# Aikku93/ulc-codec

Measured on AMD Instinct MI355X. Metric: encode+decode Msamples/s at BlockSize=2048 stereo (channel-samples through encode+decode, VBR -50, 32 blocks per stream per call), higher is better.
Workload: dtype f32; 1 GPU; vbr50 (configs[1] encode, configs[2] decode): Batch=4096 independent 44.1 kHz stereo streams/GPU x 32 blocks, BlockSize=2048, VBR -50; step = encode then decode; config=vbr50, mode=both, streams_per_gpu=4096, block_size=2048, channels=2, parallelism=batch split over 1 GPU(s), no collective on the data path

## Files before the change

### include/ulc_amd.h

```cpp
#ifndef ULC_AMD_H
#define ULC_AMD_H
#include <stddef.h>
#include <stdint.h>

#ifdef __cplusplus
extern "C" {
#endif

#ifndef ULC_AMD_NO_DROPIN_TYPES
struct ULC_TransientData_t { float Sum, SumW; };

struct ULC_EncoderState_t {
    int    RateHz;
    int    nChan;
    int    BlockSize;
    int    WindowCtrl;
    int    NextWindowCtrl;
    float  BlockComplexity;
    float  TransientFilter[3];
    void  *BufferData;
    float *SampleBuffer;
    float *TransformBuffer;
    float *TransformNoise;
    float *TransformFwdLap;
// ... 118 lines not shown
int  ulcx_encoder_reset_streams_dev(ulcx_encoder *enc, const int32_t *d_slots, int n, void *hipStream);
int  ulcx_encoder_save_streams_dev (ulcx_encoder *enc, const int32_t *d_slots, int n, uint8_t *d_state, void *hipStream);
int  ulcx_encoder_load_streams_dev (ulcx_encoder *enc, const int32_t *d_slots, int n, const uint8_t *d_state, void *hipStream);
int  ulcx_decoder_reset_streams_dev(ulcx_decoder *dec, const int32_t *d_slots, int n, void *hipStream);
int  ulcx_decoder_save_streams_dev (ulcx_decoder *dec, const int32_t *d_slots, int n, uint8_t *d_state, void *hipStream);
int  ulcx_decoder_load_streams_dev (ulcx_decoder *dec, const int32_t *d_slots, int n, const uint8_t *d_state, void *hipStream);
int  ulcx_encode_dev_subset      (ulcx_encoder *enc, const int32_t *d_slots, int n, int mode, float param0, float param1,
                                  const ulcx_rate *d_rate, const float *d_pcm , int nBlocks,
                                  uint8_t *d_out , int32_t *d_bits, int32_t *d_wc, float *d_cplx, void *hipStream);
int  ulcx_encode_dev_pcm16_subset(ulcx_encoder *enc, const int32_t *d_slots, int n, int mode, float param0, float param1,
                                  const ulcx_rate *d_rate, const int16_t *d_pcm16, int nBlocks,
                                  uint8_t *d_out, int32_t *d_bits, int32_t *d_wc, float *d_cplx, void *hipStream);
int  ulcx_analyse_dev_subset     (ulcx_encoder *enc, const int32_t *d_slots, int n, const float *d_pcm, int nBlocks,
                                  int32_t *d_wc, float *d_cplx, void *hipStream);
int  ulcx_decode_dev_subset      (ulcx_decoder *dec, const int32_t *d_slots, int n, const uint8_t *d_in ,
                                  int slotBytes, int nBlocks, float *d_pcm, int32_t *d_bits, void *hipStream);
int  ulcx_decode_dev_pcm16_subset(ulcx_decoder *dec, const int32_t *d_slots, int n, const uint8_t *d_in,
                                  int slotBytes, int nBlocks, int16_t *d_pcm16, int32_t *d_bits, void *hipStream);
int  ulcx_encoder_reset_streams_host(ulcx_encoder *enc, const int32_t *h_slots, int n);
int  ulcx_encoder_save_streams_host (ulcx_encoder *enc, const int32_t *h_slots, int n, uint8_t *h_state);
int  ulcx_encoder_load_streams_host (ulcx_encoder *enc, const int32_t *h_slots, int n, const uint8_t *h_state);
int  ulcx_decoder_reset_streams_host(ulcx_decoder *dec, const int32_t *h_slots, int n);
int  ulcx_decoder_save_streams_host (ulcx_decoder *dec, const int32_t *h_slots, int n, uint8_t *h_state);
int  ulcx_decoder_load_streams_host (ulcx_decoder *dec, const int32_t *h_slots, int n, const uint8_t *h_state);
int  ulcx_encode_host_subset(ulcx_encoder *enc, const int32_t *h_slots, int n, int mode, float param0, float param1,
                             const ulcx_rate *h_rate, const float *h_pcm, int nBlocks,
                             uint8_t *h_out, int32_t *h_bits, int32_t *h_wc, float *h_cplx);
int  ulcx_decode_host_subset(ulcx_decoder *dec, const int32_t *h_slots, int n, const uint8_t *h_in, int slotBytes, int nBlocks,
                             float *h_pcm, int32_t *h_bits);
#define ULCX_STATE_MAGIC_ENC 0x45535855u
#define ULCX_STATE_MAGIC_DEC 0x44535855u

#define ULCX_ULC_MAGIC 0x32434C55u
typedef struct ulcx_file_header {
    uint32_t Magic;
    uint16_t BlockSize;
    uint16_t MaxBlockSize;
    uint32_t nBlocks;
    uint32_t RateHz;
    uint16_t nChan;
    uint16_t RateKbps;
    uint32_t StreamOffs;
} ulcx_file_header;
void ulcx_ulc_header_pack(uint8_t dst[24], const ulcx_file_header *h);
int  ulcx_ulc_header_parse(ulcx_file_header *h, const uint8_t *src, size_t len);
int  ulcx_ulc_rate_kbps(uint64_t totalBytes, uint32_t RateHz, uint32_t BlockSize, uint32_t nBlocks);

int  ulcx_pack_streams_dev(int device, int nStreams, int nBlocks, int slotBytes, const uint8_t *d_slots, const int32_t *d_bits,
                           uint8_t *d_payload, long long payloadStride, int32_t *d_payloadBytes, int32_t *d_maxBlock, void *hipStream);

int  ulcx_decode_packed_dev(ulcx_decoder *dec, const uint8_t *d_payload, long long payloadStride, const int32_t *d_payloadBytes,
                            int nBlocks, float *d_pcm, int32_t *d_bits, void *hipStream);
int  ulcx_decode_packed_host(ulcx_decoder *dec, const uint8_t *h_payload, long long payloadStride, const int32_t *h_payloadBytes,
                             int nBlocks, float *h_pcm, int32_t *h_bits);

int  ulcx_decoder_upload_payload(ulcx_decoder *dec, const uint8_t *h_payload, long long payloadStride, const int32_t *h_payloadBytes);
int  ulcx_decode_resident_host(ulcx_decoder *dec, int nBlocks, float *h_pcm, int32_t *h_bits);

typedef struct ulcx_index_entry { int32_t ByteOffs; uint32_t RngState; } ulcx_index_entry;
int  ulcx_index_packed_dev(ulcx_decoder *dec, const uint8_t *d_payload, long long payloadStride, const int32_t *d_payloadBytes,
                           int maxBlocks, ulcx_index_entry *d_index , int32_t *d_nBlocks ,
                           void *hipStream);
int  ulcx_index_packed_host(ulcx_decoder *dec, const uint8_t *h_payload, long long payloadStride, const int32_t *h_payloadBytes,
                            int maxBlocks, ulcx_index_entry *h_index, int32_t *h_nBlocks);
int  ulcx_decode_range_dev(ulcx_decoder *dec, const uint8_t *d_payload, long long payloadStride, const int32_t *d_payloadBytes,
                           const ulcx_index_entry *d_index, int indexStride, const int32_t *d_indexBlocks,
                           const int32_t *d_first , int nBlocks,
                           float *d_pcm, int32_t *d_bits, void *hipStream);
int  ulcx_decode_range_dev_pcm16(ulcx_decoder *dec, const uint8_t *d_payload, long long payloadStride, const int32_t *d_payloadBytes,
                                 const ulcx_index_entry *d_index, int indexStride, const int32_t *d_indexBlocks,
                                 const int32_t *d_first, int nBlocks,
                                 int16_t *d_pcm16 , int32_t *d_bits, void *hipStream);
int  ulcx_decode_range_host(ulcx_decoder *dec, const uint8_t *h_payload, long long payloadStride, const int32_t *h_payloadBytes,
                            const ulcx_index_entry *h_index, int indexStride, const int32_t *h_indexBlocks,
                            const int32_t *h_first, int nBlocks, float *h_pcm, int32_t *h_bits);
int  ulcx_decoder_index_resident(ulcx_decoder *dec, int maxBlocks, int32_t *h_nBlocks);
int  ulcx_decode_resident_range_host(ulcx_decoder *dec, const int32_t *h_first, int nBlocks, float *h_pcm, int32_t *h_bits);

int  ulcx_encoder_stage_ms(ulcx_encoder *enc, float *ms, int maxStages);
int  ulcx_encoder_set_timing(ulcx_encoder *enc, int on);
int  ulcx_decoder_set_timing(ulcx_decoder *dec, int on);
const char *ulcx_encoder_stage_name(int stage);
int  ulcx_encoder_last_xf_launches(ulcx_encoder *enc);
int  ulcx_decoder_stage_ms(ulcx_decoder *dec, float *ms, int maxStages);
const char *ulcx_decoder_stage_name(int stage);

#ifdef __cplusplus
}
#endif
#endif
```

### ulc-codec_amd/csrc/ulcx_api.cpp

```cpp
#include <math.h>
#include <stdarg.h>
#include <stddef.h>
#include <stdio.h>
#include <stdlib.h>
#include <string.h>
#include <algorithm>
#include <vector>
#include "ulcx_internal.h"
#include "ulcx_rng_tables.h"


#define CKR(x) do { hipError_t e_ = (x); if (e_ != hipSuccess) { ulcx_set_error("%s: %s", #x, hipGetErrorString(e_)); return ULCX_ERR_HIP; } } while (0)
static int refuse(const char *who, const char *fmt, ...) {
    char why[384];
    va_list ap;
    va_start(ap, fmt);
    vsnprintf(why, sizeof(why), fmt, ap);
    va_end(ap);
    ulcx_set_error("%s: %s", who, why);
    return ULCX_ERR_ARG;
}

struct Block1Graph {
    hipStream_t stream = nullptr; hipGraph_t graph = nullptr; hipGraphExec_t exec = nullptr;
    bool graphed = false, noGraph = false;
};
static void block1_drop(Block1Graph &g) { if (g.graphed) { hipGraphExecDestroy(g.exec); hipGraphDestroy(g.graph); g.graphed = false; } }
template <class F> static int block1_run(Block1Graph &g, F enqueue) {
    if (!g.graphed && !g.noGraph) {
        bool ok = hipStreamBeginCapture(g.stream, hipStreamCaptureModeThreadLocal) == hipSuccess;
        if (ok) {
            const int rc = enqueue();
            hipGraph_t gr = nullptr;
            const hipError_t ee = hipStreamEndCapture(g.stream, &gr);
            ok = (rc == ULCX_OK) && ee == hipSuccess && gr != nullptr;
            if (ok) ok = hipGraphInstantiate(&g.exec, gr, nullptr, nullptr, 0) == hipSuccess;
            if (ok) { g.graph = gr; g.graphed = true; }
            else if (gr) hipGraphDestroy(gr);
        }
        if (!ok) { (void)hipGetLastError(); g.noGraph = true; }
    }
    if (g.graphed) CKR(hipGraphLaunch(g.exec, g.stream));
    else { int rc = enqueue(); if (rc) return rc; }
    CKR(hipStreamSynchronize(g.stream));
    return ULCX_OK;
}

struct ulcx_encoder {
    int device = 0, B = 0, C = 0, BS = 0, rate = 0, maxK = 0;
    UlcxEncCtx ctx = {};
    void *tables = nullptr;
    std::vector<void *> allocs;
    hipEvent_t ev[ULCX_ENC_STAGES + 1] = {};
    bool evOk = false, evRecorded = false, timing = true;
    int lastK = 0;
    UlcxEncSync sync = {};
    int wcPipe = 1, nXf = 0;
    bool keysFinal = false;
    int wcSteps = -1, wcFuse = 1;
    int nsSlots = 0;
    bool lastAnalyse = false;
    int analyseKxf = 0;
    float *d_pcm = nullptr; uint8_t *d_out = nullptr; int32_t *d_bits = nullptr, *d_wc = nullptr; float *d_cplx = nullptr;
    ulcx_rate *d_rate = nullptr;
    int lastRungs = 0;
    uint8_t *ladOut = nullptr; int32_t *ladBits = nullptr; ulcx_rate *ladRate = nullptr; int ladRungs = 0;
    struct Block1Meta { int32_t bits, wc; float cplx; int32_t pad; UlcxWcState wcs; };
    Block1Graph b1; bool b1Init = false;
    int b1Mode = 0; float b1P0 = 0.0f, b1P1 = 0.0f; int b1Rekeys = 0;
    float *pinIn = nullptr; uint8_t *pinOut = nullptr; Block1Meta *pinMeta = nullptr;
    float *subHist = nullptr; UlcxWcState *subWcs = nullptr; int32_t *subSlots = nullptr;
};
struct ulcx_decoder {
    int device = 0, B = 0, C = 0, BS = 0, maxK = 0;
    UlcxDecCtx ctx = {};
    void *tables = nullptr;
    std::vector<void *> allocs;
    hipEvent_t ev[ULCX_DEC_STAGES + 1] = {};
    bool evOk = false, evRecorded = false, timing = true;
    uint8_t *d_in = nullptr; size_t d_in_bytes = 0; float *d_pcm = nullptr; int32_t *d_bits = nullptr;
    uint8_t *d_pay = nullptr; int32_t *d_payBytes = nullptr; long long payStride = 0;
    ulcx_index_entry *d_index = nullptr; int32_t *d_idxBlocks = nullptr, *d_first = nullptr; int idxStride = 0;
    int32_t *bitsScr = nullptr;
    float *lap2 = nullptr; int *lastSub2 = nullptr; uint32_t *seed2 = nullptr; int *dead2 = nullptr;
    int synSlots = 0, scratchRows = 0, lastGrid = 0, lastFull = 0; bool splitOK = false, tailCut = true, rangeEvenFirst = false;
    Block1Graph b1; bool b1Init = false; int b1Slot = 0;
    uint8_t *pinIn = nullptr; float *pinPcm = nullptr; int32_t *pinMeta = nullptr;
    uint32_t b1Seed = 0;
    bool b1SeedStale = false, inBlock1 = false;
    float *subLap[2] = {}; int *subLastSub[2] = {}; uint32_t *subSeed[2] = {}; int *subDead[2] = {}; int *subPackOff = nullptr;
    int32_t *subSlots = nullptr;
};

#ifndef ULCX_SRC_REV
#define ULCX_SRC_REV "unknown"
#endif
extern "C" const char *ulcx_build_rev(void) { return ULCX_SRC_REV; }
extern "C" int ulcx_device_count(void) {
    int n = 0;
    hipError_t e = hipGetDeviceCount(&n);
    if (e != hipSuccess) { ulcx_set_error("hipGetDeviceCount: %s", hipGetErrorString(e)); return 0; }
    return n;
}

static int validate(int C, int BS) {
    if (C < 1 || C > 255) return 0;
    if (BS < 256 || BS > 32768) return 0;
    if ((BS & (-BS)) != BS) return 0;
    return 1;
}
static int ilog2i(int x) { int r = 0; while ((1 << r) < x) r++; return r; }

enum { ULCX_ALIGN_PCM = 16, ULCX_ALIGN_PCM16 = 8, ULCX_ALIGN_RATE = 8, ULCX_ALIGN_WORD = 4 };
static bool aligned_to(const void *p, uintptr_t a) { return ((uintptr_t)p & (a - 1)) == 0; }
static int misaligned(const char *who, const char *what, const void *p, int a) {
    if (aligned_to(p, (uintptr_t)a)) return 0;
    ulcx_set_error("%s: %s (%p) is not aligned to %d bytes", who, what, p, a);
    return 1;
}

template <typename T>
static int dalloc(std::vector<void *> &v, T **p, size_t count, bool zero) {
    void *q = nullptr;
    size_t bytes = count * sizeof(T);
    if (bytes == 0) bytes = 16;
    hipError_t e = hipMalloc(&q, bytes);
    if (e != hipSuccess) { ulcx_set_error("hipMalloc(%zu bytes): %s", bytes, hipGetErrorString(e)); return ULCX_ERR_NOMEM; }
    if (zero) { e = hipMemset(q, 0, bytes); if (e != hipSuccess) { ulcx_set_error("hipMemset: %s", hipGetErrorString(e)); hipFree(q); return ULCX_ERR_HIP; } }
    v.push_back(q);
    *p = (T *)q;
    return ULCX_OK;
}
#define DA(ptr, count, zero) do { int rc_ = dalloc(e->allocs, &(ptr), (size_t)(count), zero); if (rc_) { cleanup(e); return rc_; } } while (0)
template <typename T>
static void dfree(std::vector<void *> &v, T **p) {
    if (!*p) return;
    v.erase(std::remove(v.begin(), v.end(), (void *)*p), v.end());
    hipFree((void *)*p);
    *p = nullptr;
}
template <typename T>
static int dregrow(std::vector<void *> &v, T **p, size_t count, bool zero) { dfree(v, p); return dalloc(v, p, count, zero); }
namespace { struct DevTmp { std::vector<void *> v; ~DevTmp() { for (void *p : v) hipFree(p); } template <typename T> hipError_t get(T **p, size_t bytes) { void *q = nullptr; hipError_t r = hipMalloc(&q, bytes ? bytes : 16); if (r == hipSuccess) v.push_back(q); *p = (T *)q; return r; } }; }

static int select_device(const char *who, int device) {
    int n = ulcx_device_count();
    if (n <= 0) { if (!ulcx_last_error()[0]) ulcx_set_error("no HIP device visible"); return ULCX_ERR_NO_DEVICE; }
    if (device < 0 || device >= n) return refuse(who, "device %d out of range (have %d)", device, n);
    hipError_t e = hipSetDevice(device);
    if (e != hipSuccess) { ulcx_set_error("hipSetDevice: %s", hipGetErrorString(e)); return ULCX_ERR_NO_DEVICE; }
    return ULCX_OK;
}

static const size_t kEncSyncUntimed = offsetof(UlcxEncSync, xfTiming) / sizeof(hipEvent_t);
static void enc_sync_destroy(UlcxEncSync &s) {
    hipEvent_t *ev = &s.wcStart;
    for (size_t i = 0; i < kEncSyncUntimed + 2 * ULCX_XF_MAXCH; i++) if (ev[i]) hipEventDestroy(ev[i]);
    for (hipStream_t st : { s.side, s.side2, s.side3 }) if (st) hipStreamDestroy(st);
    s = UlcxEncSync{};
}
static bool enc_sync_create(UlcxEncSync &s) {
    static_assert(offsetof(UlcxEncSync, wcStart) == 0 && offsetof(UlcxEncSync, side) == (kEncSyncUntimed + 2 * ULCX_XF_MAXCH) * sizeof(hipEvent_t), "UlcxEncSync: events, then streams");
    hipEvent_t *ev = &s.wcStart;
    bool ok = true;
    for (hipStream_t *st : { &s.side, &s.side2, &s.side3 }) ok = ok && hipStreamCreateWithFlags(st, hipStreamNonBlocking) == hipSuccess;
    for (size_t i = 0; i < kEncSyncUntimed; i++) ok = ok && hipEventCreateWithFlags(&ev[i], hipEventDisableTiming) == hipSuccess;
    for (auto &v : s.xfTiming) ok = ok && hipEventCreate(&v) == hipSuccess;
    if (!ok) { (void)hipGetLastError(); enc_sync_destroy(s); }
    return ok;
}

static void cleanup(ulcx_encoder *e) {
    if (!e) return;
    for (void *p : e->allocs) hipFree(p);
    if (e->tables) hipFree(e->tables);
    if (e->evOk) for (auto &v : e->ev) hipEventDestroy(v);
    block1_drop(e->b1);
    if (e->b1.stream) hipStreamDestroy(e->b1.stream);
    if (e->pinIn) hipHostFree(e->pinIn);
    if (e->pinOut) hipHostFree(e->pinOut);
    if (e->pinMeta) hipHostFree(e->pinMeta);
    enc_sync_destroy(e->sync);
    delete e;
}

static int enc_reset_state(ulcx_encoder *e) {
    UlcxEncCtx &c = e->ctx;
    CKR(hipMemset(c.hist, 0, sizeof(float) * (size_t)e->B * 2 * e->BS * e->C));
    std::vector<UlcxWcState> w((size_t)e->B);
    for (auto &x : w) {
        memset(&x, 0, sizeof(x));
        x.wcPrev = 0x10;
        x.wcCur  = 0x10;
    }
    CKR(hipMemcpy(c.wcs, w.data(), sizeof(UlcxWcState) * w.size(), hipMemcpyHostToDevice));
    return ULCX_OK;
}

extern "C" int ulcx_encoder_create(ulcx_encoder **out, int device, int nStreams, int nChan, int BlockSize, int RateHz, int maxBlocksPerCall) {
    const char *who = "ulcx_encoder_create";
    if (!out) return refuse(who, "no place for the object");
    *out = nullptr;
    if (!validate(nChan, BlockSize) || nStreams < 1 || maxBlocksPerCall < 1 || RateHz < 1)
        return refuse(who, "invalid encoder geometry (nStreams=%d nChan=%d BlockSize=%d RateHz=%d maxBlocks=%d)", nStreams, nChan, BlockSize, RateHz, maxBlocksPerCall);
    if (BlockSize > ULCX_MAX_BS_DEVICE) { ulcx_set_error("BlockSize %d > %d not built for the device yet", BlockSize, ULCX_MAX_BS_DEVICE); return ULCX_ERR_UNSUPPORTED; }
    int rc = select_device(who, device);
    if (rc) return rc;
    ulcx_encoder *e = new ulcx_encoder();
    e->device = device; e->B = nStreams; e->C = nChan; e->BS = BlockSize; e->rate = RateHz; e->maxK = maxBlocksPerCall;
    UlcxEncCtx &c = e->ctx;
    c.B = nStreams; c.C = nChan; c.BS = BlockSize; c.lgBS = ilog2i(BlockSize); c.maxK = maxBlocksPerCall; c.K = 0;
    c.rateHz = RateHz;
    c.slot = 2 * nChan * BlockSize + 16;
    c.unitCap = 2 * BlockSize + 32;
    c.cHP  = 1.0f - expf(-0x1.CC845Cp6f / RateHz);
    c.cBP  = 1.0f - expf(-0x1.596344p8f / RateHz);
    c.qHP  = 1.0f - expf(-0x1.CC845Cp7f / RateHz);
    c.qBP  = 1.0f - expf(-0x1.596344p8f / RateHz);
    c.cBlk = 1.0f - expf(-0x1.1AF110p-6f * BlockSize / RateHz);
    c.cplxScale = 0x1.62E430p-1f * (31 - __builtin_clz((unsigned)BlockSize));
    rc = ulcx_tables_build(&c.T, &e->tables, BlockSize, RateHz, true);
    if (rc) { cleanup(e); return rc; }
    {
        int most = 0;
        const int N = BlockSize / 2;
        for (int t = 0; t < 2; t++) {
            const short *beg = t ? c.T.pBeg[0] : c.T.nBeg[0], *end = t ? c.T.pEnd[0] : c.T.nEnd[0];
            for (int b = 0; b < ULCX_NBARK; b++) {
                if (beg[b] > end[b] || end[b] > N) most = 1 << 20;
                if (b && (beg[b] < beg[b - 1] || end[b] < end[b - 1])) most = 1 << 20;
            }
            for (int pos = 0; pos <= N; pos++) {
                int open = 0;
                for (int b = 0; b < ULCX_NBARK; b++) open += (beg[b] <= pos && pos <= end[b]) ? 1 : 0;
                if (open > most) most = open;
            }
        }
        int ring = 4;
        while (ring < most) ring *= 2;
        c.barkRing = (ring <= 8 && N % 32 == 0) ? ring : 0;
    }
    size_t B = nStreams, K = maxBlocksPerCall, NB = B * K, cb = (size_t)nChan * BlockSize;
    DA(c.hist, B * 2 * BlockSize * nChan, true);
    DA(c.wcs, B, true);
    DA(c.env, ((B + 63) / 64) * 64 * K * BlockSize, true);
    DA(c.bins, B * (K + 1) * 16, true);
    DA(c.wcArr, B * (K + 2), true);
    DA(c.coef, NB * cb, false);
    DA(c.key, NB * cb, false);
    DA(c.nsum, ((NB * nChan + 63) / 64) * 64 * (size_t)(BlockSize / 2), false);
    DA(c.amp2, ((NB + 63) / 64) * 64 * (size_t)(BlockSize / 2), false);
    DA(c.barkN, NB * nChan * 4 * ULCX_NBARK, true);
    DA(c.barkP, NB * 4 * ULCX_NBARK, true);
    if (c.barkRing) { DA(c.barkRawN, NB * nChan * ULCX_NBARK * 3, false); DA(c.barkRawP, NB * ULCX_NBARK * 3, false); DA(c.decList, NB, false); DA(c.decCount, 1, true); }
    DA(c.nnz, NB, true);
    DA(c.cplx, NB, true);
    DA(c.nout, NB, true);
    DA(c.slow, 3 * NB + 2, true);
    c.useWave = 1;
    c.useGapSums = (cb <= 16384 && nChan <= 16) ? 1 : 0;
    DA(c.gapSum, NB * cb, false);
    DA(c.tailSum, NB * nChan * 4 * 8, true);
    c.directPack = 1;
    if (const char *ev = getenv("ULCX_DIRECT_PACK")) c.directPack = (ev[0] != '0');
    c.dbgSkip = 0;
#ifdef ULCX_ABLATE
    if (const char *ev = getenv("ULCX_DBG_SKIP")) c.dbgSkip = atoi(ev);
#endif
    DA(c.cbrLo, NB, true); DA(c.cbrHi, NB, true); DA(c.cbrDone, NB, true); DA(c.cbrBudget, NB, true); DA(c.cbrLive, 1, true);
    DA(c.selWin, NB, true); DA(c.selT, NB, true); c.selPass = 0;
    { const char *ev = getenv("ULCX_SEL_PAIR"); c.selPair = ev ? atoi(ev) : 1; }
    DA(c.keep, NB * cb / 32, true);
    DA(c.fbList, NB, true);
    DA(c.fbCount, 4, true);
    DA(c.unitBuf, NB * nChan * (size_t)c.unitCap, true);
    DA(c.unitNyb, NB * nChan * 4, true);
    {
        size_t heapBytes = (cb * 8 > ULCX_HEAP_LDS_BYTES) ? (size_t)ULCX_HEAP_GRID * cb * 8 : 16;
        uint8_t *hp = nullptr;
        DA(hp, heapBytes, false);
        c.heapScratch = hp;
    }
    for (auto &v : e->ev) { if (hipEventCreate(&v) != hipSuccess) { ulcx_set_error("hipEventCreate failed"); cleanup(e); return ULCX_ERR_HIP; } }
    e->evOk = true;
    {
        const char *evs = getenv("ULCX_ASYNC_FB");
        const bool sideOk = !(evs && evs[0] == '0') && enc_sync_create(e->sync);
        e->wcPipe = sideOk ? 4 : 1;
        if (const char *pv = getenv("ULCX_WC_PIPE")) { int n = atoi(pv); if (n >= 1 && n <= ULCX_XF_MAXCH && n != 2 && (n == 1 || sideOk)) e->wcPipe = n; }
        if (const char *sv = getenv("ULCX_WC_STEPS")) e->wcSteps = atoi(sv);
    }
    if (const char *av = getenv("ULCX_ANALYSE_KXF")) e->analyseKxf = (av[0] == '1');
    e->nsSlots = c.useGapSums ? ulcx_enc_nsums_slots(BlockSize, nChan) : 0;
    if (e->nsSlots <= 0) e->nsSlots = 1024;
    DA(c.isFb, NB, true);
    DA(c.ownSlot, NB, true);
    {
        size_t slots = NB;
        size_t maxSlots = ((size_t)8 << 30) / (cb * 4);
        size_t freeB = 0, totalB = 0;
        if (hipMemGetInfo(&freeB, &totalB) == hipSuccess && freeB / 4 / (cb * 4) < maxSlots) maxSlots = freeB / 4 / (cb * 4);
        if (maxSlots < 64) maxSlots = 64;
        if (slots > maxSlots) slots = maxSlots;
        if (const char *ev = getenv("ULCX_RANK_SLOTS")) { long n = atol(ev); if (n >= 1 && (size_t)n < slots) slots = (size_t)n; }
        for (;;) {
            int rc_ = dalloc(e->allocs, &c.rankBuf, slots * cb, false);
            if (rc_ == ULCX_OK) break;
            if (rc_ != ULCX_ERR_NOMEM || slots <= 64) { cleanup(e); return rc_; }
            (void)hipGetLastError();
            slots = (slots + 1) / 2; if (slots < 64) slots = 64;
        }
        c.rankSlots = (int)slots;
    }
    rc = enc_reset_state(e);
    if (rc) { cleanup(e); return rc; }
    *out = e;
    return ULCX_OK;
}

extern "C" void ulcx_encoder_destroy(ulcx_encoder *e) { if (e) { hipSetDevice(e->device); cleanup(e); } }
extern "C" int ulcx_encoder_reset(ulcx_encoder *e) { if (!e) return refuse("ulcx_encoder_reset", "no encoder"); CKR(hipSetDevice(e->device)); return enc_reset_state(e); }
extern "C" int ulcx_encoder_slot_bytes(const ulcx_encoder *e) { return e ? e->ctx.slot : 0; }

static UlcxEncAux enc_aux(ulcx_encoder *e, int nBlocks) {
    const int wcPipe = (nBlocks >= 2 * e->wcPipe) ? e->wcPipe : (nBlocks >= 6 && e->wcPipe > 1 ? 3 : 1);
    return UlcxEncAux{ e->sync, wcPipe, e->wcSteps, e->wcFuse, e->nsSlots, e->nXf };
}

static int slots_list_bad(const char *who, const int32_t *d_slots, int n, int B) {
    if (!d_slots || n < 1 || n > B) { ulcx_set_error("%s: no slot list, or n = %d not in 1 .. nStreams = %d", who, n, B); return 1; }
    return misaligned(who, "d_slots", d_slots, ULCX_ALIGN_WORD);
}
static int slots_host_bad(const char *who, const int32_t *h_slots, int n, int B) {
    if (!h_slots || n < 1 || n > B) { ulcx_set_error("%s: no slot list, or n = %d not in 1 .. nStreams = %d", who, n, B); return 1; }
    std::vector<char> seen((size_t)B, 0);
    for (int i = 0; i < n; i++) {
        const int s = h_slots[i];
        if (s < 0 || s >= B) { ulcx_set_error("%s: entry %d is slot %d, outside 0 .. %d", who, i, s, B - 1); return 1; }
        if (seen[(size_t)s]) { ulcx_set_error("%s: slot %d is listed twice", who, s); return 1; }
        seen[(size_t)s] = 1;
    }
    return 0;
}
static int record_headers_bad(const char *who, const uint8_t *h_state, int n, size_t bytes, const uint4 &want) {
    for (int i = 0; i < n; i++) {
        uint32_t h[4];
        memcpy(h, h_state + (size_t)i * bytes, sizeof(h));
        if (h[0] != want.x || h[1] != want.y || h[2] != want.z || h[3] != want.w) {
            ulcx_set_error("%s: record %d is {magic %08x, nChan %u, BlockSize %u, RateHz %u}, this object takes {%08x, %u, %u, %u}", who, i,
                           h[0], h[1], h[2], h[3], want.x, want.y, want.z, want.w);
            return 1;
        }
    }
    return 0;
}
enum { ULCX_ALIGN_STATE = 16, ULCX_STATE_HEADER = 16, ULCX_WCS_WORDS = sizeof(UlcxWcState) / 4, ULCX_WCS_REC_BYTES = (sizeof(UlcxWcState) + 15) / 16 * 16 };
static size_t enc_hist_bytes(const ulcx_encoder *e) { return sizeof(float) * 2 * (size_t)e->BS * e->C; }
extern "C" size_t ulcx_encoder_stream_state_bytes(const ulcx_encoder *e) { return e ? ULCX_STATE_HEADER + enc_hist_bytes(e) + ULCX_WCS_REC_BYTES : 0; }
static size_t slot_state_bytes(const ulcx_encoder *e) { return ulcx_encoder_stream_state_bytes(e); }
static void slot_touch(ulcx_encoder *) {}
static UlcxSlotGeom slot_geom(const ulcx_encoder *e, bool record) {
    UlcxSlotGeom g = {};
    g.B = e->B; g.rowVec = (int)(enc_hist_bytes(e) / 16); g.isEnc = 1; g.nSmall = 1; g.smallWords = ULCX_WCS_WORDS;
    g.padWords = record ? ULCX_WCS_REC_BYTES / 4 : ULCX_WCS_WORDS;
    g.header = make_uint4(ULCX_STATE_MAGIC_ENC, (unsigned)e->C, (unsigned)e->BS, (unsigned)e->rate);
    return g;
}
static UlcxSlotRows enc_slot_rows(const ulcx_encoder *e, float *hist, UlcxWcState *wcs) {
    UlcxSlotRows r = {};
    r.big = (uint8_t *)hist; r.bigStride = enc_hist_bytes(e); r.small[0] = (uint8_t *)wcs; r.smallStride = sizeof(UlcxWcState);
    return r;
}
static UlcxSlotRows slot_obj_rows(const ulcx_encoder *e) { return enc_slot_rows(e, e->ctx.hist, e->ctx.wcs); }
static UlcxSlotRows slot_record_rows(const ulcx_encoder *e, uint8_t *state) {
    UlcxSlotRows r = {};
    const size_t bytes = slot_state_bytes(e);
    r.hdr = state; r.hdrStride = bytes; r.big = state + ULCX_STATE_HEADER; r.bigStride = bytes;
    r.small[0] = state + ULCX_STATE_HEADER + enc_hist_bytes(e); r.smallStride = bytes;
    return r;
}
static int enc_shadow(ulcx_encoder *e) {
    int rc;
    if (!e->subHist && (rc = dalloc(e->allocs, &e->subHist, (size_t)e->B * 2 * e->BS * e->C, false))) return rc;
    if (!e->subWcs && (rc = dalloc(e->allocs, &e->subWcs, (size_t)e->B, false))) return rc;
    return ULCX_OK;
}

static bool mode_ok(int m) { return m == ULCX_MODE_VBR || m == ULCX_MODE_CBR || m == ULCX_MODE_ABR; }
static int enc_args_bad(const char *who, const ulcx_encoder *e, const void *pcm, bool haveOut, int nBlocks) {
    if (!e || !pcm || !haveOut) { refuse(who, "bad argument"); return 1; }
    if (nBlocks < 1 || nBlocks > e->maxK) { refuse(who, "nBlocks out of range"); return 1; }
    return 0;
}
static int rate_entry_bad(const char *who, const char *what, int index, float r, float a) {
    if (isfinite(r) && isfinite(a) && r != 0.0f && !(a < 0.0f)) return 0;
    refuse(who, "%s %d (RateKbps %g, AvgComplexity %g)", what, index, (double)r, (double)a);
    return 1;
}
static int rate_table_bad(const char *who, const char *what, const ulcx_rate *h_rate, int n) {
    for (int i = 0; i < n; i++) if (rate_entry_bad(who, what, i, h_rate[i].RateKbps, h_rate[i].AvgComplexity)) return 1;
    return 0;
}
static UlcxEncCtx enc_call_ctx(const ulcx_encoder *e, int mode, float p0, float p1, const ulcx_rate *d_rate, const float *d_pcm, const int16_t *d_pcm16, int nBlocks) {
    UlcxEncCtx c = e->ctx;
    if (d_rate) { mode = ULCX_MODE_VBR; p0 = 100.0f; p1 = 0.0f; }
    c.K = nBlocks; c.keyFinal = 0; c.mode = mode; c.p0 = p0; c.p1 = p1;
    c.vbrTarget = (mode == ULCX_MODE_VBR) ? 0x1.E4EFB7p3f * logf(100.0f / p0) : 0.0f;
    c.rates = (const float2 *)d_rate;
    c.pcm = d_pcm; c.pcm16 = d_pcm16; c.out = nullptr; c.bits = nullptr; c.wcOut = nullptr; c.cplxOut = nullptr;
    return c;
}
static int enc_call_done(ulcx_encoder *e, int rc, int nBlocks, bool analyse, int rungs) {
    e->evRecorded = (rc == ULCX_OK) && e->timing;
    e->lastK = nBlocks;
    e->keysFinal = false;
    e->lastAnalyse = analyse;
    e->lastRungs = rungs;
    return rc;
}
template <class F> static int enc_launch_on(ulcx_encoder *e, UlcxEncCtx &c, const int32_t *d_slots, int n, hipStream_t st, F launch) {
    if (!d_slots) return launch(c);
    int rc = enc_shadow(e);
    if (rc) return rc;
    const UlcxSlotRows shadow = enc_slot_rows(e, e->subHist, e->subWcs);
    if ((rc = ulcx_slots_gather(slot_obj_rows(e), shadow, d_slots, n, slot_geom(e, false), st))) return rc;
    c.B = n; c.hist = e->subHist; c.wcs = e->subWcs;
    rc = launch(c);
    if (rc == ULCX_OK) rc = ulcx_slots_scatter(slot_obj_rows(e), shadow, d_slots, n, slot_geom(e, false), st);
    return rc;
}

static int encode_dev_any(const char *who, ulcx_encoder *e, int mode, float p0, float p1, const ulcx_rate *d_rate, bool needRate,
                          const float *d_pcm, const int16_t *d_pcm16, int nBlocks, uint8_t *d_out, int32_t *d_bits, int32_t *d_wc, float *d_cplx,
                          void *hipStream, bool subset = false, const int32_t *d_slots = nullptr, int n = 0) {
    if (enc_args_bad(who, e, d_pcm ? (const void *)d_pcm : d_pcm16, d_out && d_bits && (d_rate || !needRate), nBlocks)) return ULCX_ERR_ARG;
    if (subset && slots_list_bad(who, d_slots, n, e->B)) return ULCX_ERR_ARG;
    if (!d_rate && !mode_ok(mode)) return refuse(who, "bad mode");
    if (misaligned(who, "d_pcm", d_pcm, ULCX_ALIGN_PCM) || misaligned(who, "d_pcm16", d_pcm16, ULCX_ALIGN_PCM16) ||
        misaligned(who, "d_rate", d_rate, ULCX_ALIGN_RATE) || misaligned(who, "d_bits", d_bits, ULCX_ALIGN_WORD) ||
        misaligned(who, "d_wc", d_wc, ULCX_ALIGN_WORD) || misaligned(who, "d_cplx", d_cplx, ULCX_ALIGN_WORD)) return ULCX_ERR_ARG;
    CKR(hipSetDevice(e->device));
    UlcxEncCtx c = enc_call_ctx(e, mode, p0, p1, d_rate, d_pcm, d_pcm16, nBlocks);
    c.out = d_out; c.bits = d_bits; c.wcOut = d_wc; c.cplxOut = d_cplx;
    const UlcxEncAux aux = enc_aux(e, nBlocks);
    const int rc = enc_launch_on(e, c, subset ? d_slots : nullptr, n, (hipStream_t)hipStream,
                                 [&](UlcxEncCtx &cc) { return ulcx_enc_launch(cc, (hipStream_t)hipStream, e->timing ? e->ev : nullptr, aux); });
    return enc_call_done(e, rc, nBlocks, false, 1);
}
extern "C" int ulcx_encode_dev(ulcx_encoder *e, int mode, float p0, float p1, const float *d_pcm, int nBlocks,
                               uint8_t *d_out, int32_t *d_bits, int32_t *d_wc, float *d_cplx, void *hipStream) {
    return encode_dev_any("ulcx_encode_dev", e, mode, p0, p1, nullptr, false, d_pcm, nullptr, nBlocks, d_out, d_bits, d_wc, d_cplx, hipStream);
}
extern "C" int ulcx_encode_dev_pcm16(ulcx_encoder *e, int mode, float p0, float p1, const int16_t *d_pcm16, int nBlocks,
                                     uint8_t *d_out, int32_t *d_bits, int32_t *d_wc, float *d_cplx, void *hipStream) {
    return encode_dev_any("ulcx_encode_dev_pcm16", e, mode, p0, p1, nullptr, false, nullptr, d_pcm16, nBlocks, d_out, d_bits, d_wc, d_cplx, hipStream);
}
extern "C" int ulcx_encode_dev_rates(ulcx_encoder *e, const ulcx_rate *d_rate, const float *d_pcm, int nBlocks,
                                     uint8_t *d_out, int32_t *d_bits, int32_t *d_wc, float *d_cplx, void *hipStream) {
    return encode_dev_any("ulcx_encode_dev_rates", e, 0, 0.0f, 0.0f, d_rate, true, d_pcm, nullptr, nBlocks, d_out, d_bits, d_wc, d_cplx, hipStream);
}
extern "C" int ulcx_encode_dev_pcm16_rates(ulcx_encoder *e, const ulcx_rate *d_rate, const int16_t *d_pcm16, int nBlocks,
                                           uint8_t *d_out, int32_t *d_bits, int32_t *d_wc, float *d_cplx, void *hipStream) {
    return encode_dev_any("ulcx_encode_dev_pcm16_rates", e, 0, 0.0f, 0.0f, d_rate, true, nullptr, d_pcm16, nBlocks, d_out, d_bits, d_wc, d_cplx, hipStream);
}
extern "C" int ulcx_encode_dev_subset(ulcx_encoder *e, const int32_t *d_slots, int n, int mode, float p0, float p1, const ulcx_rate *d_rate, const float *d_pcm, int nBlocks,
                                      uint8_t *d_out, int32_t *d_bits, int32_t *d_wc, float *d_cplx, void *hipStream) {
    return encode_dev_any("ulcx_encode_dev_subset", e, mode, p0, p1, d_rate, false, d_pcm, nullptr, nBlocks, d_out, d_bits, d_wc, d_cplx, hipStream, true, d_slots, n);
}
extern "C" int ulcx_encode_dev_pcm16_subset(ulcx_encoder *e, const int32_t *d_slots, int n, int mode, float p0, float p1, const ulcx_rate *d_rate, const int16_t *d_pcm16, int nBlocks,
                                            uint8_t *d_out, int32_t *d_bits, int32_t *d_wc, float *d_cplx, void *hipStream) {
    return encode_dev_any("ulcx_encode_dev_pcm16_subset", e, mode, p0, p1, d_rate, false, nullptr, d_pcm16, nBlocks, d_out, d_bits, d_wc, d_cplx, hipStream, true, d_slots, n);
}

static int ladder_bad(const char *who, const ulcx_rung *rungs, int nRungs) {
    if (!rungs || nRungs < 1 || nRungs > ULCX_MAX_RUNGS) { refuse(who, "nRungs %d not in 1 .. %d (or no rungs)", nRungs, ULCX_MAX_RUNGS); return 1; }
    for (int r = 0; r < nRungs; r++) {
        if (rungs[r].reserved != 0) { refuse(who, "rung %d: reserved must be 0", r); return 1; }
        if (!rungs[r].rate && !mode_ok(rungs[r].mode)) { refuse(who, "rung %d: bad mode %d", r, rungs[r].mode); return 1; }
    }
    return 0;
}
static int encode_ladder_any(const char *who, ulcx_encoder *e, const ulcx_rung *rungs, int nRungs, const float *d_pcm, const int16_t *d_pcm16, int nBlocks,
                             uint8_t *d_out, int32_t *d_bits, int32_t *d_wc, float *d_cplx, void *hipStream) {
    if (ladder_bad(who, rungs, nRungs) || enc_args_bad(who, e, d_pcm ? (const void *)d_pcm : d_pcm16, d_out && d_bits, nBlocks)) return ULCX_ERR_ARG;
    if (misaligned(who, "d_pcm", d_pcm, ULCX_ALIGN_PCM) || misaligned(who, "d_pcm16", d_pcm16, ULCX_ALIGN_PCM16) ||
        misaligned(who, "d_bits", d_bits, ULCX_ALIGN_WORD) || misaligned(who, "d_wc", d_wc, ULCX_ALIGN_WORD) ||
        misaligned(who, "d_cplx", d_cplx, ULCX_ALIGN_WORD)) return ULCX_ERR_ARG;
    for (int r = 0; r < nRungs; r++) if (misaligned(who, "a rung's rate table", rungs[r].rate, ULCX_ALIGN_RATE)) return ULCX_ERR_ARG;
    CKR(hipSetDevice(e->device));
    UlcxEncCtx cs[ULCX_MAX_RUNGS];
    const size_t NB = (size_t)e->B * nBlocks;
    for (int r = 0; r < nRungs; r++) {
        UlcxEncCtx &c = cs[r];
        c = enc_call_ctx(e, rungs[r].mode, rungs[r].param0, rungs[r].param1, rungs[r].rate, d_pcm, d_pcm16, nBlocks);
        c.out = d_out + r * NB * (size_t)c.slot; c.bits = d_bits + r * NB;
        if (!r) { c.wcOut = d_wc; c.cplxOut = d_cplx; }
    }
    const int rc = ulcx_enc_launch_ladder(cs, nRungs, (hipStream_t)hipStream, e->timing ? e->ev : nullptr, enc_aux(e, nBlocks));
    return enc_call_done(e, rc, nBlocks, false, nRungs);
}
extern "C" int ulcx_encode_dev_ladder(ulcx_encoder *e, const ulcx_rung *rungs, int nRungs, const float *d_pcm, int nBlocks,
                                      uint8_t *d_out, int32_t *d_bits, int32_t *d_wc, float *d_cplx, void *hipStream) {
    return encode_ladder_any("ulcx_encode_dev_ladder", e, rungs, nRungs, d_pcm, nullptr, nBlocks, d_out, d_bits, d_wc, d_cplx, hipStream);
}
extern "C" int ulcx_encode_dev_pcm16_ladder(ulcx_encoder *e, const ulcx_rung *rungs, int nRungs, const int16_t *d_pcm16, int nBlocks,
                                            uint8_t *d_out, int32_t *d_bits, int32_t *d_wc, float *d_cplx, void *hipStream) {
    return encode_ladder_any("ulcx_encode_dev_pcm16_ladder", e, rungs, nRungs, nullptr, d_pcm16, nBlocks, d_out, d_bits, d_wc, d_cplx, hipStream);
}
extern "C" int ulcx_encoder_last_rungs(ulcx_encoder *e) { return e ? e->lastRungs : refuse("ulcx_encoder_last_rungs", "no encoder"); }

static int analyse_dev_any(const char *who, ulcx_encoder *e, const float *d_pcm, const int16_t *d_pcm16, int nBlocks, int32_t *d_wc, float *d_cplx, void *hipStream,
                           bool subset = false, const int32_t *d_slots = nullptr, int n = 0) {
    if (enc_args_bad(who, e, d_pcm ? (const void *)d_pcm : d_pcm16, d_wc || d_cplx, nBlocks)) return ULCX_ERR_ARG;
    if (subset && slots_list_bad(who, d_slots, n, e->B)) return ULCX_ERR_ARG;
    if (misaligned(who, "d_pcm", d_pcm, ULCX_ALIGN_PCM) || misaligned(who, "d_pcm16", d_pcm16, ULCX_ALIGN_PCM16) ||
        misaligned(who, "d_wc", d_wc, ULCX_ALIGN_WORD) || misaligned(who, "d_cplx", d_cplx, ULCX_ALIGN_WORD)) return ULCX_ERR_ARG;
    CKR(hipSetDevice(e->device));
    UlcxEncCtx c = enc_call_ctx(e, ULCX_MODE_VBR, 100.0f, 0.0f, nullptr, d_pcm, d_pcm16, nBlocks);
    c.wcOut = d_wc; c.cplxOut = d_cplx;
    const UlcxEncAux aux = enc_aux(e, nBlocks);
    const int rc = enc_launch_on(e, c, subset ? d_slots : nullptr, n, (hipStream_t)hipStream,
                                 [&](UlcxEncCtx &cc) { return ulcx_analyse_launch(cc, (hipStream_t)hipStream, e->timing ? e->ev : nullptr, aux, e->analyseKxf); });
    return enc_call_done(e, rc, nBlocks, true, 0);
}
extern "C" int ulcx_analyse_dev(ulcx_encoder *e, const float *d_pcm, int nBlocks, int32_t *d_wc, float *d_cplx, void *hipStream) {
    return analyse_dev_any("ulcx_analyse_dev", e, d_pcm, nullptr, nBlocks, d_wc, d_cplx, hipStream);
}
extern "C" int ulcx_analyse_dev_pcm16(ulcx_encoder *e, const int16_t *d_pcm16, int nBlocks, int32_t *d_wc, float *d_cplx, void *hipStream) {
    return analyse_dev_any("ulcx_analyse_dev_pcm16", e, nullptr, d_pcm16, nBlocks, d_wc, d_cplx, hipStream);
}
// ... 143 lines not shown
        if (++e->b1Rekeys >= 2) e->b1.noGraph = true;
    }
    if (!e->b1.graphed) { e->b1Mode = mode; e->b1P0 = p0; e->b1P1 = p1; }
    { int rc = block1_run(e->b1, enqueue); if (rc) return rc; }
    const int32_t nb = e->pinMeta->bits;
    memcpy(h_out, e->pinOut, (nb > 0 && (size_t)(nb + 7) / 8 <= slot) ? (size_t)(nb + 7) / 8 : slot);
    if (bits) *bits = nb;
    if (cplx) *cplx = e->pinMeta->cplx;
    if (stateOut) { stateOut[0] = e->pinMeta->wcs.wcPrev; stateOut[1] = e->pinMeta->wcs.wcCur; }
    if (transientFilter) for (int i = 0; i < 3; i++) transientFilter[i] = e->pinMeta->wcs.tf[i];
    return ULCX_OK;
}

extern "C" int ulcx_encoder_debug_fetch(ulcx_encoder *e, int nBlocks, float *h_coef, float *h_noise, float *h_keys, uint8_t *h_keep, int32_t *h_nout) {
    const char *who = "ulcx_encoder_debug_fetch";
    if (!e || nBlocks < 1 || nBlocks > e->maxK) return refuse(who, "no encoder, or nBlocks out of range");
    if (e->lastAnalyse) return refuse(who, "the last call was an analysis call (no intermediates)");
    CKR(hipSetDevice(e->device));
    CKR(hipDeviceSynchronize());
    size_t NB = (size_t)e->B * nBlocks, cb = (size_t)e->C * e->BS;
    if (h_coef)  CKR(hipMemcpy(h_coef, e->ctx.coef, sizeof(float) * NB * cb, hipMemcpyDeviceToHost));
    if (h_noise) {
        if (!e->ctx.npair) { int rc = dalloc(e->allocs, &e->ctx.npair, (size_t)e->B * e->maxK * cb, false); if (rc) return rc; }
        UlcxEncCtx c2 = e->ctx; c2.K = nBlocks;
        ulcx_enc_materialise_noise(c2, nullptr);
        CKR(hipDeviceSynchronize());
        CKR(hipMemcpy(h_noise, e->ctx.npair, sizeof(float) * NB * cb, hipMemcpyDeviceToHost));
    }
    if (h_keys) {
        if (!e->keysFinal) {
            UlcxEncCtx c2 = e->ctx; c2.K = nBlocks; c2.keyFinal = 0;
            ulcx_enc_finalize_keys(c2, nullptr);
            CKR(hipDeviceSynchronize());
            e->keysFinal = true;
        }
        CKR(hipMemcpy(h_keys, e->ctx.key, sizeof(float) * NB * cb, hipMemcpyDeviceToHost));
    }
    if (h_nout)  CKR(hipMemcpy(h_nout, e->ctx.nout, sizeof(int32_t) * NB, hipMemcpyDeviceToHost));
    if (h_keep) {
        std::vector<uint32_t> bits(NB * cb / 32);
        CKR(hipMemcpy(bits.data(), e->ctx.keep, sizeof(uint32_t) * bits.size(), hipMemcpyDeviceToHost));
        for (size_t i = 0; i < NB * cb; i++) h_keep[i] = (bits[i >> 5] >> (i & 31)) & 1;
    }
    return ULCX_OK;
}

extern "C" int ulcx_encoder_debug_force_exact(ulcx_encoder *e, int every) {
    if (!e || every < 0) return refuse("ulcx_encoder_debug_force_exact", "no encoder, or every < 0");
    e->ctx.forceFb = every;
    return ULCX_OK;
}
extern "C" int ulcx_encoder_last_fallbacks(ulcx_encoder *e) {
    if (!e) return refuse("ulcx_encoder_last_fallbacks", "no encoder");
    if (e->lastAnalyse) return 0;
    CKR(hipSetDevice(e->device));
    CKR(hipDeviceSynchronize());
    int n[2] = { 0, 0 };
    CKR(hipMemcpy(n, e->ctx.fbCount, sizeof(n), hipMemcpyDeviceToHost));
    return n[0] + (e->lastRungs > 1 ? n[1] : 0);
}
extern "C" const char *ulcx_encoder_stage_name(int i) { return (i >= 0 && i < ULCX_ENC_STAGES_REPORTED) ? ulcx_enc_stage_names[i] : ""; }
extern "C" int ulcx_encoder_stage_ms(ulcx_encoder *e, float *ms, int maxStages) {
    if (!e || !e->evRecorded) return 0;
    int n = 0;
    for (int i = 0; i < ULCX_ENC_STAGES && i < maxStages; i++) {
        float t = 0;
        if (hipEventElapsedTime(&t, e->ev[i], e->ev[i + 1]) != hipSuccess) break;
        ms[n++] = (e->lastAnalyse && i > 6 && i < ULCX_ENC_STAGES - 1) ? 0.0f : t;
    }
    if (n == ULCX_ENC_STAGES && n < maxStages) {
        const int IX_XF = 5;
        float exposed = 0.0f;
        if (e->nXf > 0) {
            float sum = 0.0f; bool ok = true;
            for (int j = 0; j < e->nXf; j++) { float t = 0; if (hipEventElapsedTime(&t, e->sync.xfTiming[2 * j], e->sync.xfTiming[2 * j + 1]) != hipSuccess) { ok = false; break; } sum += t; }
            if (ok) { exposed = ms[IX_XF] - sum; ms[IX_XF] = sum; }
        }
        ms[n++] = exposed;
    }
    return n;
}

extern "C" int ulcx_encoder_last_xf_launches(ulcx_encoder *e) { return (e && e->evRecorded) ? (e->nXf > 0 ? e->nXf : 1) : 0; }

static void cleanup(ulcx_decoder *e) {
    if (!e) return;
    for (void *p : e->allocs) hipFree(p);
    if (e->tables) hipFree(e->tables);
    if (e->evOk) for (auto &v : e->ev) hipEventDestroy(v);
    block1_drop(e->b1);
    if (e->b1.stream) hipStreamDestroy(e->b1.stream);
    if (e->pinIn) hipHostFree(e->pinIn);
    if (e->pinPcm) hipHostFree(e->pinPcm);
    if (e->pinMeta) hipHostFree(e->pinMeta);
    delete e;
}
static int dec_reset_state(ulcx_decoder *e) {
    UlcxDecCtx &c = e->ctx;
    CKR(hipMemset(c.lap, 0, sizeof(float) * (size_t)e->B * e->C * (e->BS / 2)));
    CKR(hipMemset(c.lastSub, 0, sizeof(int) * (size_t)e->B));
    CKR(hipMemset(c.dead, 0, sizeof(int) * (size_t)e->B));
    CKR(hipMemset(c.packOff, 0, sizeof(int) * (size_t)e->B));
    std::vector<uint32_t> seed((size_t)e->B, 1234567u);
    CKR(hipMemcpy(c.seed, seed.data(), sizeof(uint32_t) * seed.size(), hipMemcpyHostToDevice));
    e->b1Seed = 1234567u; e->b1SeedStale = false; e->inBlock1 = false;
    return ULCX_OK;
}

extern "C" int ulcx_dec_split_plan(int nStreams, int nBlocks, int residentWG) {
    if (nStreams < 1 || nBlocks < 1 || residentWG < 1) return 0;
    const long long T = (long long)nStreams * nBlocks;
    long long per = (T + residentWG - 1) / residentWG; if (per < 8) per = 8;
    const long long grid = T / per;
    const long long costStream = (((long long)nStreams + residentWG - 1) / residentWG) * nBlocks;
    return (grid >= 1 && grid != nStreams && (per + 1) * 3 < costStream * 2) ? (int)grid : 0;
}
#define ULCX_DSYN_TAIL_LEN 8
extern "C" int ulcx_dec_tail_plan(int nStreams, int nBlocks, int residentWG, int *full) {
    if (full) *full = 0;
    if (nStreams < 1 || nBlocks < 3 * ULCX_DSYN_TAIL_LEN || residentWG < 1) return 0;
    const int rem = nStreams % residentWG;
    if (rem == 0 || (long long)rem * 5 > (long long)residentWG * 4) return 0;
    const int len = nBlocks / 4 > ULCX_DSYN_TAIL_LEN ? nBlocks / 4 : ULCX_DSYN_TAIL_LEN;
    const long long n = (long long)rem * nBlocks / len;
    if (full) *full = nStreams - rem;
    return (int)n;
}
extern "C" int ulcx_dec_range_tail_plan(int nStreams, int nBlocks, int residentWG, int *full) {
    if (nBlocks >= 3 * ULCX_DSYN_TAIL_LEN) return ulcx_dec_tail_plan(nStreams, nBlocks, residentWG, full);
    if (full) *full = 0;
    if (nStreams < 1 || nBlocks < 1 || residentWG < 1 || nStreams <= residentWG) return 0;
    const int len = nBlocks / 4 > 2 ? nBlocks / 4 : 2;
    if (nBlocks < 3 * len) return 0;
    const int rem = nStreams % residentWG;
    if (rem == 0 || (long long)rem * 5 > (long long)residentWG * 4) return 0;
    if (full) *full = nStreams - rem;
    return (int)((long long)rem * nBlocks / len);
}
extern "C" int ulcx_decoder_last_cut(ulcx_decoder *e, int *workgroups, int *wholeStreams, int *residentWG) {
    if (!e) return refuse("ulcx_decoder_last_cut", "no decoder");
    if (workgroups) *workgroups = e->lastGrid;
    if (wholeStreams) *wholeStreams = e->lastFull;
    if (residentWG) *residentWG = e->synSlots;
    return ULCX_OK;
}
static int dec_launch(ulcx_decoder *e, UlcxDecCtx &c, hipStream_t st, int *subsetSet = nullptr) {
    if (!e->inBlock1) e->b1SeedStale = true;
    UlcxDecAux a;
    a.synGrid = 0; a.synFull = 0;
    c.lapO = c.lap; c.lastSubO = c.lastSub; c.seedO = c.seed; c.deadO = c.dead;
    const int Kc = c.range ? c.K - 1 : c.K;
    if (e->splitOK && e->synSlots > 0) {
        if (c.range && c.B > e->synSlots && e->tailCut && !e->rangeEvenFirst) {
            int full = 0;
            const int tail = ulcx_dec_range_tail_plan(c.B, Kc, e->synSlots, &full);
            if (tail > 0 && tail <= e->scratchRows) { a.synGrid = full + tail; a.synFull = full; }
        }
        if (!a.synGrid) a.synGrid = ulcx_dec_split_plan(c.B, Kc, e->synSlots);
        if (!a.synGrid) {
            int full = 0;
            const int tail = c.range ? ulcx_dec_range_tail_plan(c.B, Kc, e->synSlots, &full) : ulcx_dec_tail_plan(c.B, Kc, e->synSlots, &full);
            if (tail > 0 && tail <= e->scratchRows && e->tailCut) { a.synGrid = full + tail; a.synFull = full; }
        }
        if (a.synGrid) {
            if (getenv("ULCX_DEBUG_PRINT")) fprintf(stderr, "[ulcx] synthesis: %lld (stream, block) pairs over %d workgroups (%d of them one stream each; %d resident)\n", (long long)c.B * Kc, a.synGrid, a.synFull, e->synSlots);
            if (subsetSet) { c.lapO = e->subLap[1]; c.lastSubO = e->subLastSub[1]; c.seedO = e->subSeed[1]; c.deadO = e->subDead[1]; }
// ... 569 lines not shown
```

### ulc-codec_amd/csrc/ulcx_enc.hip

```cpp
#include "ulcx_enc_dev.h"

static size_t ulcx_enc_xf_lds_bytes(int BS, int C) {
    if (BS > 8192) return (size_t)BS * 4;
    int ps = ulcx_xf_pad_shift(BS, C);
    size_t z = (size_t)4 * (BS + (BS >> ps)) * 4;
    size_t full = z + (size_t)BS * 2 + 32 + (C > 2 ? (size_t)BS * 2 : 0);
    return full <= ULCX_LDS_LIMIT ? full : z + (size_t)BS * 2 + 32;
}

static size_t ulcx_enc_xfa_lds_bytes(int BS, int C) {
    if (BS > 8192) return (size_t)BS * 4;
    int ps = ulcx_xf_pad_shift(BS, C);
    return (size_t)2 * (BS + (BS >> ps)) * 4 + (size_t)BS * 2 + 32;
}

#define CK(x) do { hipError_t e_ = (x); if (e_ != hipSuccess) { ulcx_set_error("%s: %s", #x, hipGetErrorString(e_)); return ULCX_ERR_HIP; } } while (0)
#define TRY(x) do { int rc_ = (x); if (rc_) return rc_; } while (0)

typedef void (*RangeKernel)(UlcxEncCtx, int, int);
typedef void (*PassKernel)(UlcxEncCtx, int);
typedef void (*CallKernel)(UlcxEncCtx);

static RangeKernel wc_energy_fn(const UlcxEncCtx &c) { return c.pcm16 ? k_wc_energy<int16_t> : k_wc_energy<float>; }
static RangeKernel wc_ef_fn(const UlcxEncCtx &c) { return c.pcm16 ? k_wc_ef<EF_NW, int16_t> : k_wc_ef<EF_NW, float>; }
static CallKernel state_update_fn(const UlcxEncCtx &c) { return c.pcm16 ? k_state_update<int16_t> : k_state_update<float>; }

template <typename IN> static RangeKernel xf_fn_in(const UlcxEncCtx &c, bool mdctOnly) {
    if (c.BS > 8192) return mdctOnly ? k_xfa_big<IN> : k_xf_big<IN>;
    if (c.C == 2) return mdctOnly ? k_xfa<true, IN> : k_xf<true, IN>;
    return mdctOnly ? k_xfa<false, IN> : k_xf<false, IN>;
}
static RangeKernel xf_fn(const UlcxEncCtx &c, bool mdctOnly) { return c.pcm16 ? xf_fn_in<int16_t>(c, mdctOnly) : xf_fn_in<float>(c, mdctOnly); }

template <int PASS> static PassKernel select_fn_pass(const UlcxEncCtx &c, bool pair, bool rates) {
#define SEL(R, L) (rates ? (PassKernel)k_select_wave_rates<R, L, PASS> : (PassKernel)k_select_wave<R, L, PASS>)
    switch (c.C * c.BS / 64) {
        case 128:
            if (pair) return rates ? k_select_pair_rates<64, 12, PASS> : k_select_pair<64, 12, PASS>;
            return SEL(128, 0);
        case 64: return c.lgBS == 11 ? SEL(64, 11) : SEL(64, 0);
        case 32: return SEL(32, 0);
        case 16: return SEL(16, 0);
        case 8:  return SEL(8, 0);
        case 4:  return SEL(4, 0);
        default: return nullptr;
    }
#undef SEL
}
static PassKernel select_fn(const UlcxEncCtx &c, bool pair, bool rates, int pass) {
    return pass == 1 ? select_fn_pass<1>(c, pair, rates) : pass == 2 ? select_fn_pass<2>(c, pair, rates) : select_fn_pass<0>(c, pair, rates);
}

static int allow_lds(const void *fn, size_t lds) {
    if (lds > 48 * 1024) CK(hipFuncSetAttribute(fn, hipFuncAttributeMaxDynamicSharedMemorySize, (int)lds));
    return ULCX_OK;
}

static void launch_wc_energy(const UlcxEncCtx &c, unsigned grid, hipStream_t st, int k0, int k1) {
    hipLaunchKernelGGL(wc_energy_fn(c), dim3(grid), dim3(WG), 0, st, c, k0, k1);
}

static void launch_wc_ef(const UlcxEncCtx &c, hipStream_t st, int k0, int k1) {
    static_assert(EF_LDS_BYTES <= 48 * 1024, "k_wc_ef: raise the dynamic LDS limit with hipFuncSetAttribute");
    hipLaunchKernelGGL(wc_ef_fn(c), dim3((c.B + EF_SPW - 1) / EF_SPW), dim3(EF_NW * 64), EF_LDS_BYTES, st, c, k0, k1);
}

static void launch_state_update(const UlcxEncCtx &c, hipStream_t st) {
    hipLaunchKernelGGL(state_update_fn(c), dim3(c.B), dim3(WG), 0, st, c);
}

const char *const ulcx_enc_stage_names[ULCX_ENC_STAGES_REPORTED] = {
    "k_wc_energy", "k_wc_forward", "k_wc_backward", "k_wc_integrate", "k_wc_decide",
    "k_xf", "k_cplx", "k_pbark", "k_mask",
    "k_select", "k_nbark", "(k_nline: gone)", "k_heapsel", "k_nsums", "k_tails", "k_encode_wave", "k_encode_units", "k_pack", "cbr_probe_passes", "k_state_update", "wc_pipeline_exposed",
};

struct StageMarks { hipEvent_t *ev; int stage; };
#define MARK(mk, s) do { if ((mk).ev) CK(hipEventRecord((mk).ev[(mk).stage++], s)); } while (0)

enum { ULCX_FRONT_ENCODE = 0, ULCX_FRONT_ANALYSE = 1, ULCX_FRONT_ANALYSE_KXF = 2, ULCX_FRONT_WC_ONLY = 3 };
static int launch_front(const UlcxEncCtx &c, hipStream_t st, StageMarks &mk, const UlcxEncAux &aux, const int what) {
    UlcxEncSync &sy = aux.sync;
    hipStream_t side = sy.side, side2 = sy.side2, side3 = sy.side3;
    const int SG = (c.B + 63) / 64;
    const int nCh = aux.wcPipe;
    const bool mdctOnly = (what == ULCX_FRONT_ANALYSE);
    const RangeKernel xf = (what == ULCX_FRONT_WC_ONLY) ? nullptr : xf_fn(c, mdctOnly);
    const size_t lds = mdctOnly ? ulcx_enc_xfa_lds_bytes(c.BS, c.C) : ulcx_enc_xf_lds_bytes(c.BS, c.C);
    if (xf) TRY(allow_lds((const void *)xf, lds));
    auto transform = [&](int k0, int k1) {
        if (xf) hipLaunchKernelGGL(xf, dim3((unsigned)((c.B * (k1 - k0) + 7) / 8) * 8), dim3(WG), lds, st, c, k0, k1);
    };
    const bool wcFuse = c.C == 2 && aux.wcFuse;
    aux.nXf = 0;
    if (nCh <= 1) {
        if (wcFuse) { MARK(mk, st); launch_wc_ef(c, st, 0, c.K);                                                  MARK(mk, st); }
        else {
        launch_wc_energy(c, (unsigned)(SG * ((c.K * c.BS) / 64)), st, 0, c.K);                                    MARK(mk, st);
        hipLaunchKernelGGL(k_wc_forward, dim3((c.B * 2 + 63) / 64), dim3(64), 0, st, c, 0, c.K);                  MARK(mk, st);
        }
        hipLaunchKernelGGL(k_wc_backward, dim3(SG * c.K), dim3(64), 0, st, c, 0, c.K);                            MARK(mk, st);
        hipLaunchKernelGGL(k_wc_integrate, dim3((c.B + 63) / 64), dim3(64), 0, st, c, 0, c.K);                    MARK(mk, st);
        hipLaunchKernelGGL(k_wc_decide, dim3((c.B * c.K + 63) / 64), dim3(64), 0, st, c, 0, c.K);                 MARK(mk, st);
        transform(0, c.K);
        MARK(mk, st);
        return ULCX_OK;
    }
    for (int i = 0; i < 5; i++) MARK(mk, st);
    int nW = aux.wcSteps;
    if (nW < 0) nW = (c.K >= 8) ? 4 : 0;
    if (nW > ULCX_WC_MAXCH) nW = ULCX_WC_MAXCH;
    if (nW > c.K) nW = c.K;
    const bool sameCuts = nW < 1;
    if (sameCuts) nW = nCh;
    int cut[ULCX_XF_MAXCH + 1];
    cut[0] = 0; cut[1] = 1;
    for (int j = 2; j <= nCh; j++) cut[j] = 1 + (c.K - 1) * (j - 1) / (nCh - 1);
    int wcs[ULCX_WC_MAXCH + 1];
    for (int w = 0; w <= nW; w++) wcs[w] = sameCuts ? cut[w] : (int)((long long)c.K * w / nW);
    CK(hipEventRecord(sy.wcStart, st));
    CK(hipStreamWaitEvent(side, sy.wcStart, 0));
    int jx = 0;
    for (int w = 0; w < nW; w++) {
        const int k0 = wcs[w], k1 = wcs[w + 1], kc = k1 - k0;
        if (wcFuse) launch_wc_ef(c, side, k0, k1);
        else {
            launch_wc_energy(c, (unsigned)(SG * ((kc * c.BS) / 64)), side, k0, k1);
            hipLaunchKernelGGL(k_wc_forward, dim3((c.B * 2 + 63) / 64), dim3(64), 0, side, c, k0, k1);
        }
        CK(hipEventRecord(sy.wcForward[w], side));
        CK(hipStreamWaitEvent(side2, sy.wcForward[w], 0));
        hipLaunchKernelGGL(k_wc_backward, dim3(SG * kc), dim3(64), 0, side2, c, k0, k1);
        CK(hipEventRecord(sy.wcBackward[w], side2));
        CK(hipStreamWaitEvent(side3, sy.wcBackward[w], 0));
        hipLaunchKernelGGL(k_wc_integrate, dim3((c.B + 63) / 64), dim3(64), 0, side3, c, k0, k1);
        hipLaunchKernelGGL(k_wc_decide, dim3((c.B * kc + 63) / 64), dim3(64), 0, side3, c, k0, k1);
        CK(hipEventRecord(sy.wcDecided[w], side3));
        while (jx < nCh && cut[jx + 1] <= k1) {
            CK(hipStreamWaitEvent(st, sy.wcDecided[w], 0));
            if (mk.ev) CK(hipEventRecord(sy.xfTiming[2 * jx], st));
            if (!(ULCX_DBG(c) & 0x2000))
            transform(cut[jx], cut[jx + 1]);
            if (mk.ev) CK(hipEventRecord(sy.xfTiming[2 * jx + 1], st));
            CK(hipEventRecord(sy.xfChunkDone[jx], st));
            jx++;
        }
    }
    aux.nXf = nCh;
    MARK(mk, st);
    for (int j = 0; j < nCh; j++) {
        CK(hipStreamWaitEvent(side, sy.xfChunkDone[j], 0));
        const int kc2 = cut[j + 1] - cut[j];
        if (what == ULCX_FRONT_ENCODE) hipLaunchKernelGGL(k_cplx, dim3((c.B * kc2 + 63) / 64), dim3(64), 0, side, c, cut[j], cut[j + 1]);
        else hipLaunchKernelGGL(k_cplxa, dim3((c.B * kc2 + 63) / 64), dim3(64), 0, side, c, cut[j], cut[j + 1]);
    }
    CK(hipEventRecord(sy.cplxChunksDone, side));
    return ULCX_OK;
}

struct EncPlan {
    int NB, N, nUnits;
    bool aside;
    int probes;
    size_t barkLds;
    bool selWave, selPair;
    size_t selLds;
    int ldsEntries, fbGrid; size_t heapLds;
    WaveCaps capS, capM, capF;
    bool haveFull, haveMid;
    int nsSlots;
};
static int enc_probes(const UlcxEncCtx &c, int N) {
    int n = 0;
    if (c.mode != ULCX_MODE_VBR || c.rates != nullptr) { n = 2; for (int m = N; m > 1; m >>= 1) n++; }
    return n;
}
static EncPlan enc_plan(const UlcxEncCtx &c, const UlcxEncAux &aux) {
    EncPlan p;
    p.NB = c.B * c.K; p.N = c.C * c.BS; p.nUnits = p.NB * c.C * 4;
    p.aside = aux.sync.side != nullptr;
    p.probes = enc_probes(c, p.N);
    p.barkLds = (size_t)c.barkRing * 3 * 64 * 8 + (size_t)2 * BK_TILE_FLOATS * 4;
    const int R = p.N / 64;
    p.selWave = (R == 4 || R == 8 || R == 16 || R == 32 || R == 64 || R == 128);
    p.selPair = (R == 128 && c.C == 2 && c.selPair);
    p.selLds = (size_t)(p.selPair ? 1 : 4) * ulcx_sel_lds_words(c.BS) * sizeof(float);
    p.ldsEntries = ((size_t)p.N * 8 <= ULCX_HEAP_LDS_BYTES) ? p.N : 0;
    p.heapLds = p.ldsEntries ? (size_t)p.N * 8 + (size_t)p.N / 8 : 0;
    p.fbGrid = p.NB < ULCX_HEAP_GRID ? p.NB : ULCX_HEAP_GRID;
    p.capS = { WAVE_SK, WAVE_SZ, WAVE_SN };
    p.capF = { (c.BS + 63) & ~63, ((c.BS / 2) + 63) & ~63, 4 * c.BS + 64 };
    while ((size_t)wavecaps_lds(p.capF) * 4 > 150 * 1024) {
        p.capF.k = (p.capF.k / 2 + 63) & ~63; p.capF.z = (p.capF.z / 2 + 63) & ~63; p.capF.nyb = p.capF.nyb / 2 + 32;
    }
    p.haveFull = p.capF.k > p.capS.k;
    p.capM = { 1024, 512, 4096 };
    p.haveMid = p.capM.k < p.capF.k;
    p.nsSlots = aux.nsSlots;
    return p;
}

static void launch_noise(const UlcxEncCtx &c, const EncPlan &p, hipStream_t s2) {
    if (c.barkRing) {
        hipLaunchKernelGGL(k_bark_uniform<true>, dim3((p.NB * c.C + 63) / 64), dim3(256), p.barkLds, s2, c);
        hipLaunchKernelGGL(k_bark_levels<true>, dim3((unsigned)(((size_t)p.NB * c.C * 32 + WG - 1) / WG)), dim3(WG), 0, s2, c);
    }
    hipLaunchKernelGGL(k_nbark, dim3((p.nUnits + 63) / 64), dim3(64), 0, s2, c, c.barkRing ? 1 : 0);
}

static int launch_psy(const UlcxEncCtx &c, const EncPlan &p, UlcxEncSync &sy, hipStream_t st, StageMarks &mk, bool cplxChunked) {
    if (c.barkRing) { TRY(allow_lds((const void *)k_bark_uniform<true>, p.barkLds)); TRY(allow_lds((const void *)k_bark_uniform<false>, p.barkLds)); }
    if (p.aside) {
        CK(hipEventRecord(sy.noiseFork, st));
        CK(hipStreamWaitEvent(sy.side3, sy.noiseFork, 0));
        if (cplxChunked) CK(hipStreamWaitEvent(sy.side3, sy.cplxChunksDone, 0));
        else hipLaunchKernelGGL(k_cplx, dim3((p.NB + 63) / 64), dim3(64), 0, sy.side3, c, 0, c.K);
        CK(hipEventRecord(sy.cplxDone, sy.side3));
        MARK(mk, st);
        launch_state_update(c, sy.side3);
        CK(hipEventRecord(sy.stateDone, sy.side3));
        CK(hipStreamWaitEvent(sy.side2, sy.noiseFork, 0));
        launch_noise(c, p, sy.side2);
        CK(hipEventRecord(sy.noiseDone, sy.side2));
    } else { hipLaunchKernelGGL(k_cplx, dim3((p.NB + 63) / 64), dim3(64), 0, st, c, 0, c.K);                MARK(mk, st); }
    const bool uniP = c.barkRing != 0;
    if (uniP) {
        hipLaunchKernelGGL(k_bark_uniform<false>, dim3((p.NB + 63) / 64), dim3(256), p.barkLds, st, c);
        hipLaunchKernelGGL(k_bark_levels<false>, dim3((unsigned)(((size_t)p.NB * 32 + WG - 1) / WG)), dim3(WG), 0, st, c);
    }
    hipLaunchKernelGGL(k_pbark, dim3((p.NB * 4 + 63) / 64), dim3(64), 0, st, c, uniP ? 1 : 0);            MARK(mk, st);
    MARK(mk, st);
    if (p.aside) CK(hipStreamWaitEvent(st, sy.cplxDone, 0));
    return ULCX_OK;
}

static int launch_select_wave(const UlcxEncCtx &c, const EncPlan &p, hipStream_t st, bool rates, int pass, int fin) {
    const PassKernel fn = select_fn(c, p.selPair, rates, pass);
    TRY(allow_lds((const void *)fn, p.selLds));
// ... 169 lines not shown
```

### ulc-codec_amd/csrc/ulcx_enc_dev.h

```cpp
#pragma once
#include <utility>
#include "ulcx_internal.h"

#include <type_traits>

#include "ulcx_libm.h"

#define WG 256

#define FFT_PACKED

#include "ulcx_fft.h"

__device__ __forceinline__ float fastlog(float x) {
    uint32_t b = __float_as_uint(x);
    int e = (int)(b >> 23) - 127;
    float m = __uint_as_float((127u << 23) | (b & 0x7FFFFFu));
    return -1.7417939f + (2.8212026f + (-1.4699568f + (0.44717955f - 0.056570851f * m) * m) * m) * m + 0.6931471806f * e;
}

__device__ __forceinline__ int quant_u(float v) {
    return (v >= 0.5f) ? (int)(0.5f + sqrtf(v - 0.25f)) : 0;
}

// ... 272 lines not shown
    asm volatile("" : "+v"(k));
    return (fabsf(re) < 0.5f * ULCX_COEF_EPS) ? __uint_as_float(0xff800000u) : k;
}

__device__ __forceinline__ uint32_t sel_key(float re, float m, int ch) {
    float k = fastlog(re * re);
    asm("" : "+v"(k));
    k = (fabsf(re) < 0.5f * ULCX_COEF_EPS) ? __uint_as_float(0xff800000u) : k;
    float t = __builtin_fmaf(k, 2.0f, m);
    if (ch & 1) t = t + -0x1.62E430p0f;
    const uint32_t u = __float_as_uint(t);
    return u ^ ((uint32_t)((int32_t)u >> 31) | 0x80000000u);
}

#define E_GAPCAP(N) ((N) / 16)

#define WAVE_SYNC_E() do { __builtin_amdgcn_fence(__ATOMIC_RELEASE, "wavefront"); __builtin_amdgcn_wave_barrier(); __builtin_amdgcn_fence(__ATOMIC_ACQUIRE, "wavefront"); } while (0)

#ifndef NSUMS_LB

#define NSUMS_LB 8

#endif

__host__ __device__ static inline size_t nsums_lds_bytes(int N, int C) {
    return (size_t)N * 4 + N / 8 + 8 * (size_t)E_GAPCAP(N) + 16 + 8 * (size_t)((N / 32 + 63) / 64) + (size_t)C * 4 * ULCX_NBARK * 4 + 32 * 8 + N / 16;
}

#define TAILS_U 64

#define TAILS_TP 8

struct WaveCaps { int k, z, nyb; };

#ifndef WAVE_SK
#define WAVE_SK 512
#endif
#ifndef WAVE_SZ
#define WAVE_SZ 128
#endif
#ifndef WAVE_SN
#define WAVE_SN 1280
#endif

__host__ __device__ static inline int wavecaps_lds(const WaveCaps &w) { return w.k * 4 + w.z * 8 + w.k * 4 + w.z + w.nyb + 64; }

__device__ __forceinline__ int wave_excl_scan(int v, int lane, int &total) {
    int x = v;
#define STEP(ctl, rmask) x += __builtin_amdgcn_update_dpp(0, x, ctl, rmask, 0xf, false);
    ULCX_DPP_STEPS(STEP)
#undef STEP
    total = __builtin_amdgcn_readlane(x, 63);
    (void)lane;
    return x - v;
}

#define WAVE_SYNC() do { __builtin_amdgcn_fence(__ATOMIC_RELEASE, "wavefront"); __builtin_amdgcn_wave_barrier(); __builtin_amdgcn_fence(__ATOMIC_ACQUIRE, "wavefront"); } while (0)

#define XCH_WORD(total, last, fail, seq) ((unsigned long long)((uint32_t)(total) | ((uint32_t)(last) << 16) | ((uint32_t)(fail) << 20)) | ((unsigned long long)(uint32_t)(seq) << 32))

template <typename IN>
__global__ __launch_bounds__(WG) void k_wc_energy(UlcxEncCtx c, int k0, int k1);
extern template __global__ void k_wc_energy<float>(UlcxEncCtx, int, int);
extern template __global__ void k_wc_energy<int16_t>(UlcxEncCtx, int, int);
__global__ void k_wc_forward(UlcxEncCtx c, int k0, int k1);
template <int NW, typename IN>
__global__ __launch_bounds__(NW * 64) void k_wc_ef(UlcxEncCtx c, int k0, int k1);
extern template __global__ void k_wc_ef<EF_NW, float>(UlcxEncCtx, int, int);
extern template __global__ void k_wc_ef<EF_NW, int16_t>(UlcxEncCtx, int, int);
__global__ void k_wc_backward(UlcxEncCtx c, int k0, int k1);
__global__ void k_wc_integrate(UlcxEncCtx c, int k0, int k1);
__global__ void k_wc_decide(UlcxEncCtx c, int k0, int k1);
template <bool ST, typename IN>
__global__ __launch_bounds__(WG, 4) void k_xf(UlcxEncCtx c, int k0, int k1);
extern template __global__ void k_xf<false, float>(UlcxEncCtx, int, int);
extern template __global__ void k_xf<false, int16_t>(UlcxEncCtx, int, int);
extern template __global__ void k_xf<true, float>(UlcxEncCtx, int, int);
extern template __global__ void k_xf<true, int16_t>(UlcxEncCtx, int, int);
template <typename IN>
__global__ __launch_bounds__(WG) void k_xf_big(UlcxEncCtx c, int k0, int k1);
extern template __global__ void k_xf_big<float>(UlcxEncCtx, int, int);
extern template __global__ void k_xf_big<int16_t>(UlcxEncCtx, int, int);
__global__ void k_cplx(UlcxEncCtx c, int k0, int k1);
#ifndef XFA_LB
#define XFA_LB 4
#endif
template <bool ST, typename IN>
__global__ __launch_bounds__(WG, XFA_LB) void k_xfa(UlcxEncCtx c, int k0, int k1);
extern template __global__ void k_xfa<false, float>(UlcxEncCtx, int, int);
extern template __global__ void k_xfa<false, int16_t>(UlcxEncCtx, int, int);
extern template __global__ void k_xfa<true, float>(UlcxEncCtx, int, int);
extern template __global__ void k_xfa<true, int16_t>(UlcxEncCtx, int, int);
template <typename IN>
__global__ __launch_bounds__(WG) void k_xfa_big(UlcxEncCtx c, int k0, int k1);
extern template __global__ void k_xfa_big<float>(UlcxEncCtx, int, int);
extern template __global__ void k_xfa_big<int16_t>(UlcxEncCtx, int, int);
__global__ void k_cplxa(UlcxEncCtx c, int k0, int k1);
__global__ void k_nbark(UlcxEncCtx c, int useList);
__global__ void k_nline(UlcxEncCtx c);
__global__ void k_pbark(UlcxEncCtx c, int useList);
template <bool NOISE>
__global__ __launch_bounds__(256) void k_bark_uniform(UlcxEncCtx c);
extern template __global__ void k_bark_uniform<false>(UlcxEncCtx);
extern template __global__ void k_bark_uniform<true>(UlcxEncCtx);
template <bool NOISE>
__global__ __launch_bounds__(WG) void k_bark_levels(UlcxEncCtx c);
extern template __global__ void k_bark_levels<false>(UlcxEncCtx);
extern template __global__ void k_bark_levels<true>(UlcxEncCtx);
__global__ void k_keys_finalize(UlcxEncCtx c);
__global__ void k_select(UlcxEncCtx c, int finalPass);
#define SEL_MINW(R, LGBS, PASS) ((R) >= 128 ? 2 : ((R) == 64 && !((LGBS) == 11 && (PASS) == 0)) ? 5 : 6)
template <int R, int LGBS = 0, int PASS = 0>
__global__ __launch_bounds__(256, SEL_MINW(R, LGBS, PASS)) void k_select_wave(UlcxEncCtx c, int finalPass);
extern template __global__ void k_select_wave<128, 0, 0>(UlcxEncCtx, int);
extern template __global__ void k_select_wave<128, 0, 1>(UlcxEncCtx, int);
extern template __global__ void k_select_wave<128, 0, 2>(UlcxEncCtx, int);
extern template __global__ void k_select_wave<16, 0, 0>(UlcxEncCtx, int);
extern template __global__ void k_select_wave<16, 0, 1>(UlcxEncCtx, int);
extern template __global__ void k_select_wave<16, 0, 2>(UlcxEncCtx, int);
extern template __global__ void k_select_wave<32, 0, 0>(UlcxEncCtx, int);
extern template __global__ void k_select_wave<32, 0, 1>(UlcxEncCtx, int);
extern template __global__ void k_select_wave<32, 0, 2>(UlcxEncCtx, int);
extern template __global__ void k_select_wave<4, 0, 0>(UlcxEncCtx, int);
extern template __global__ void k_select_wave<4, 0, 1>(UlcxEncCtx, int);
extern template __global__ void k_select_wave<4, 0, 2>(UlcxEncCtx, int);
extern template __global__ void k_select_wave<64, 0, 0>(UlcxEncCtx, int);
extern template __global__ void k_select_wave<64, 0, 1>(UlcxEncCtx, int);
extern template __global__ void k_select_wave<64, 0, 2>(UlcxEncCtx, int);
extern template __global__ void k_select_wave<64, 11, 0>(UlcxEncCtx, int);
extern template __global__ void k_select_wave<64, 11, 1>(UlcxEncCtx, int);
extern template __global__ void k_select_wave<64, 11, 2>(UlcxEncCtx, int);
extern template __global__ void k_select_wave<8, 0, 0>(UlcxEncCtx, int);
extern template __global__ void k_select_wave<8, 0, 1>(UlcxEncCtx, int);
extern template __global__ void k_select_wave<8, 0, 2>(UlcxEncCtx, int);
template <int R, int LGBS = 0, int PASS = 0>
__global__ __launch_bounds__(128) void k_select_pair(UlcxEncCtx c, int finalPass);
extern template __global__ void k_select_pair<64, 12, 0>(UlcxEncCtx, int);
extern template __global__ void k_select_pair<64, 12, 1>(UlcxEncCtx, int);
extern template __global__ void k_select_pair<64, 12, 2>(UlcxEncCtx, int);
template <int R, int LGBS = 0, int PASS = 0>
__global__ __launch_bounds__(256, SEL_MINW(R, LGBS, PASS)) void k_select_wave_rates(UlcxEncCtx c, int finalPass);
template <int R, int LGBS = 0, int PASS = 0>
__global__ __launch_bounds__(128) void k_select_pair_rates(UlcxEncCtx c, int finalPass);
#define ULCX_SEL_RATES_EXT(R, L) extern template __global__ void k_select_wave_rates<R, L, 0>(UlcxEncCtx, int); \
                                 extern template __global__ void k_select_wave_rates<R, L, 1>(UlcxEncCtx, int); \
                                 extern template __global__ void k_select_wave_rates<R, L, 2>(UlcxEncCtx, int);
ULCX_SEL_RATES_EXT(128, 0) ULCX_SEL_RATES_EXT(64, 0) ULCX_SEL_RATES_EXT(64, 11) ULCX_SEL_RATES_EXT(32, 0)
ULCX_SEL_RATES_EXT(16, 0) ULCX_SEL_RATES_EXT(8, 0) ULCX_SEL_RATES_EXT(4, 0)
#undef ULCX_SEL_RATES_EXT
extern template __global__ void k_select_pair_rates<64, 12, 0>(UlcxEncCtx, int);
extern template __global__ void k_select_pair_rates<64, 12, 1>(UlcxEncCtx, int);
extern template __global__ void k_select_pair_rates<64, 12, 2>(UlcxEncCtx, int);
__global__ void k_heapsel(UlcxEncCtx c, int ldsEntries);
__global__ void k_heapsel_pipe(UlcxEncCtx c, int fullRanking);
__global__ void k_keep_ranks(UlcxEncCtx c, int finalPass);
__global__ void k_nsums(UlcxEncCtx c, int finalPass);
__global__ void k_tails(UlcxEncCtx c, int finalPass);
__global__ void k_encode_units(UlcxEncCtx c, int finalPass);
#ifndef EW_LB
#define EW_LB 6
#endif
template <bool SMALL>
__global__ __launch_bounds__(256, SMALL ? EW_LB : 1) void k_encode_wave(UlcxEncCtx c, int finalPass, WaveCaps caps, int phase);
extern template __global__ void k_encode_wave<false>(UlcxEncCtx, int, WaveCaps, int);
extern template __global__ void k_encode_wave<true>(UlcxEncCtx, int, WaveCaps, int);
__global__ void k_rate_step(UlcxEncCtx c);
// ... 6 lines not shown
```

### ulc-codec_amd/csrc/ulcx_enc_xf.hip

```cpp
#include "ulcx_enc_dev.h"

__device__ __forceinline__ int first_overlap(int wc, int BS) {
    unsigned p = ulcx_pattern(wc);
    int ov = BS >> (p & 7);
    if (p & 8) ov >>= (wc & 7);
    return ov;
}

__device__ __forceinline__ float win_apply(float x, int i, int S, int aL, int ovL, int aR, int ov,
                                           const float *__restrict__ rise, const float *__restrict__ fall) {
    if (i < S) return (i < aL) ? 0.0f : (i < aL + ovL) ? x * rise[i - aL] : x;
    int n = i - S;
    return (n < aR) ? x : (n < aR + ov) ? x * fall[n - aR] : 0.0f;
}

template <typename IN, int BSC, bool AN = false>
__device__ __forceinline__ int xf_fast(const UlcxEncCtx &c, float *lds, int s, int k, int blk, int tid) {
    constexpr int BS = BSC, S = BSC, M = BSC / 2, PS = 4, Mp = FFT_PADDEDS(M, PS);
    constexpr int LGM = BSC == 4096 ? 11 : 10;
    static_assert(BSC == 2048 || BSC == 4096, "sizes with a compile-time transform");
    static_assert(WG == 256 && (M / 2) % (2 * WG) == 0, "whole fold / epilogue trips per thread");
    float2 *z = (float2 *)lds;
    float2 *twl = (float2 *)(lds + (AN ? 2 : 4) * FFT_PADDEDS(BS, PS));
    float2 *zc0 = z, *zs0 = z + Mp, *zc1 = z + (AN ? 1 : 2) * Mp, *zs1 = z + 3 * Mp;
    const float2 *pre = c.T.pre[0];
    const float *rise = c.T.winRise + S, *fall = c.T.winFall + S;
    const IN *pcmS = pcm_base<IN>(c) + (size_t)s * c.K * BS * 2;
    const IN *frameLo = pcmS + (ptrdiff_t)(k - 2) * BS * 2, *frameHi = frameLo;
    if constexpr (std::is_same<IN, float>::value) {
        const float *histS = c.hist + (size_t)s * 2 * BS * 2;
        if (k < 2) frameLo = histS + (size_t)k * BS * 2;
        if (k < 1) frameHi = histS;
    }
#pragma unroll
    for (int i = tid; i < M / 2; i += WG) twl[i] = c.T.tw[0][i];
#pragma unroll
    for (int jj0 = 0; jj0 < M / 2; jj0 += WG) {
        const int jj = jj0 + tid;
        const int iA = 2 * jj, iB = S - 2 - 2 * jj, iC = S + 2 * jj, iD = 2 * S - 2 - 2 * jj;
        const int ip[4] = { iA, iB, iC, iD };
        float2 xs[8];
#pragma unroll
        for (int r = 0; r < 4; r++) {
            const float4 v = ld4((r < 2 ? frameLo : frameHi) + (size_t)ip[r] * 2);
            const float2 m0 = make_float2((v.x + v.y) * 0.5f, (v.x - v.y) * 0.5f);
            const float2 m1 = make_float2((v.z + v.w) * 0.5f, (v.z - v.w) * 0.5f);
            const float2 fw = (r < 2) ? *(const float2 *)(rise + ip[r]) : *(const float2 *)(fall + ip[r] - S);
            xs[2 * r]     = make_float2(m0.x * fw.x, m0.y * fw.x);
            xs[2 * r + 1] = make_float2(m1.x * fw.y, m1.y * fw.y);
        }
#pragma unroll
        for (int hsel = 0; hsel < 2; hsel++) {
            const int n = hsel ? M / 2 + jj : M / 2 - 1 - jj;
            const float2 lbv = hsel ? xs[0] : xs[1], lav = hsel ? xs[3] : xs[2];
            const float2 rav = hsel ? xs[4] : xs[5], rbv = hsel ? xs[7] : xs[6];
            const float2 P = pre[n];
#pragma unroll
            for (int q = 0; q < 2; q++) {
                const float ra = q ? rav.y : rav.x, rb = q ? rbv.y : rbv.x, la = q ? lav.y : lav.x, lb = q ? lbv.y : lbv.x;
                const float vr = ra + rb, wr = ra - rb;
                const float vl = la - lb, wl = lb + la;
                const float v1 = hsel ? vl : vr, v2 = hsel ? vr : vl;
                const float w1 = hsel ? wl : wr, w2 = hsel ? wr : wl;
                float2 *zc = q ? zc1 : zc0, *zs = q ? zs1 : zs0;
                zc[FFT_PADS(n, PS)] = cmulc(make_float2(v1, v2), P);
                if constexpr (!AN) zs[FFT_PADS(n, PS)] = cmulc(make_float2(w2, w1), P);
            }
        }
    }
    __syncthreads();
    if constexpr (AN) { if (tid < 128) fft_wave_dif_ct<M, PS>(z + __builtin_amdgcn_readfirstlane(tid >> 6) * Mp, twl, tid & 63); }
    else fft_wave_dif_ct<M, PS>(z + __builtin_amdgcn_readfirstlane(tid >> 6) * Mp, twl, tid & 63);
    __syncthreads();
    float *coefO = c.coef + (size_t)blk * (2 * BS);
    constexpr float norm = 2.0f / S;
    int nnz = 0;
    if constexpr (AN) {
#pragma unroll
        for (int e0 = 0; e0 < M / 2; e0 += 2 * WG) {
            const int kA = e0 + 2 * tid, kB = e0 + 2 * tid + 1;
            const int kk2[2] = { kA, kB };
            float re[2][2][4];
#pragma unroll
// ... 11 lines not shown
#pragma unroll
                    for (int p = 0; p < 2; p++) {
                        const int slot = p ? (1 - u) : u;
                        re[q][p][2 * slot] = mdct[2*p] * norm; re[q][p][2 * slot + 1] = mdct[2*p+1] * norm;
                    }
                }
            }
            const int j1 = kA, j2 = M - 1 - kB;
#pragma unroll
            for (int q = 0; q < 2; q++) {
                stnt((float4 *)(coefO + q * BS + 2 * j1), make_float4(re[q][0][0], re[q][0][1], re[q][0][2], re[q][0][3]));
                stnt((float4 *)(coefO + q * BS + 2 * j2), make_float4(re[q][1][0], re[q][1][1], re[q][1][2], re[q][1][3]));
            }
        }
        return 0;
    }
#pragma unroll
    for (int e0 = 0; e0 < M / 2; e0 += 2 * WG) {
        const int kA = e0 + 2 * tid, kB = e0 + 2 * tid + 1;
        const int kk2[2] = { kA, kB };
        float re[2][2][4];
        float ns[2][2][2];
        float am[2][2] = { { 0.0f, 0.0f }, { 0.0f, 0.0f } };
#pragma unroll
        for (int u = 0; u < 2; u++) {
            const int k1 = kk2[u], k2 = M - 1 - k1;
            const int r1 = (int)(__brev((unsigned)k1) >> (32 - LGM)), r2 = (int)(__brev((unsigned)k2) >> (32 - LGM));
            const float2 P1 = pre[k1], P2 = pre[k2];
            const fft_v2f Pv1 = { P1.x, P1.y }, Pv2 = { P2.x, P2.y };
#pragma unroll
            for (int q = 0; q < 2; q++) {
                const float2 *zc = q ? zc1 : zc0, *zs = q ? zs1 : zs0;
                auto cm = [](float2 d, fft_v2f w) { const fft_v2f dv = { d.x, d.y }; const fft_v2f r = fft_cmulc_post_pk(dv, w); return make_float2(r.x, r.y); };
                const float2 yc1 = cm(zc[FFT_PADS(r1, PS)], Pv1), yc2 = cm(zc[FFT_PADS(r2, PS)], Pv2);
                const float2 ys1 = cm(zs[FFT_PADS(r1, PS)], Pv1), ys2 = cm(zs[FFT_PADS(r2, PS)], Pv2);
                const float mdct[4] = { yc1.x, yc2.y, yc2.x, yc1.y };
                const float mdst[4] = { ys1.x, ys2.y, ys2.x, ys1.y };
#pragma unroll
                for (int p = 0; p < 2; p++) {
                    const float re0 = mdct[2*p] * norm,   im0 = mdst[2*p] * norm;
                    const float re1 = mdct[2*p+1] * norm, im1 = mdst[2*p+1] * norm;
                    const float re0s = re0 * re0, im0s = im0 * im0, re1s = re1 * re1, im1s = im1 * im1;
                    const float a0 = re0s + im0s, a1 = re1s + im1s;
                    nnz += (fabsf(re0) < 0.5f * ULCX_COEF_EPS) ? 0 : 1;
                    nnz += (fabsf(re1) < 0.5f * ULCX_COEF_EPS) ? 0 : 1;
                    const int slot = p ? (1 - u) : u;
                    re[q][p][2 * slot] = re0; re[q][p][2 * slot + 1] = re1;
                    ns[q][p][slot] = a0 + a1;
                    am[p][slot] += a0; am[p][slot] += a1;
                }
            }
        }
        const int j1 = kA, j2 = M - 1 - kB;
#pragma unroll
        for (int q = 0; q < 2; q++) {
            stnt((float4 *)(coefO + q * BS + 2 * j1), make_float4(re[q][0][0], re[q][0][1], re[q][0][2], re[q][0][3]));
            stnt((float4 *)(coefO + q * BS + 2 * j2), make_float4(re[q][1][0], re[q][1][1], re[q][1][2], re[q][1][3]));
            stnt((float2 *)(c.nsum + tile_idx(BS / 2, blk * 2 + q, j1)), make_float2(ns[q][0][0], ns[q][0][1]));
            stnt((float2 *)(c.nsum + tile_idx(BS / 2, blk * 2 + q, j2)), make_float2(ns[q][1][0], ns[q][1][1]));
        }
        *(float2 *)(c.amp2 + tile_idx(BS / 2, blk, j1)) = make_float2(am[0][0], am[0][1]);
        *(float2 *)(c.amp2 + tile_idx(BS / 2, blk, j2)) = make_float2(am[1][0], am[1][1]);
    }
    return nnz;
}

template <typename IN>
__device__ __forceinline__ bool xf_is_fast(const UlcxEncCtx &c, int s, int k) {
#ifdef XF_NO_FAST
    return false;
#endif
    const int BS = c.BS;
    const int *wrow = c.wcArr + (size_t)s * (c.maxK + 2) + k;
    const int wcPrev = wrow[0], wc = wrow[1], wcNext = wrow[2];
    if (!(k >= 2 || std::is_same<IN, float>::value) || (ulcx_pattern(wc) >> 4) != 0) return false;
    unsigned pp = ulcx_pattern(wcPrev);
    int lastS = BS;
    do { lastS = BS >> (pp & 7); } while (pp >>= 4);
    int ovFirst = first_overlap(wc, BS);
    if (ovFirst > lastS) ovFirst = lastS;
    return ovFirst == BS && first_overlap(wcNext, BS) >= BS;
}

template <bool ST, typename IN, bool AN = false>
__device__ __forceinline__ void xf_block(const UlcxEncCtx &c, float *lds, int s, int k, const int tid) {
    const int BS = c.BS, C = ST ? 2 : c.C;
    const int blk = s * c.K + k;
    const int ps = ulcx_xf_pad_shift(BS, C);
    float2 *z    = (float2 *)lds;
    constexpr int NA = AN ? 2 : 4;
    float2 *twl  = (float2 *)(lds + NA * FFT_PADDEDS(BS, ps));
    int    &s_nnz = *(int *)(lds + NA * FFT_PADDEDS(BS, ps) + BS / 2);
    const bool ampLds = !AN && (C > 2);
    const bool twInLds = !(ampLds && (size_t)16 * (BS + (BS >> ps)) + (size_t)BS * 4 + 32 > ULCX_LDS_LIMIT);
    float  *amp2 = twInLds ? lds + 4 * FFT_PADDEDS(BS, ps) + BS / 2 + 4 : lds + 4 * FFT_PADDEDS(BS, ps);
    if (!AN && tid == 0) s_nnz = 0;
    if (ampLds) for (int i = tid; i < BS / 2; i += WG) amp2[i] = 0.0f;

    const int *wrow = c.wcArr + (size_t)s * (c.maxK + 2) + k;
    int wcPrev = wrow[0], wc = wrow[1], wcNext = wrow[2];
    if (!AN && c.barkRing && tid == 0 && (ulcx_pattern(wc) & ~8u) != 0) c.decList[atomicAdd(c.decCount, 1)] = blk;
    int nextOv = first_overlap(wcNext, BS);
    int ovFirst;
    {
        unsigned pp = ulcx_pattern(wcPrev);
        int lastS = BS;
        do { lastS = BS >> (pp & 7); } while (pp >>= 4);
        ovFirst = first_overlap(wc, BS);
        if (ovFirst > lastS) ovFirst = lastS;
    }
    size_t cb = (size_t)C * BS;
    float *coefO = c.coef + (size_t)blk * cb;
    int nnz = 0;
    __syncthreads();

#ifdef XF_NO_FAST
    const bool fastBlk = false;
#else
    const bool fastBlk = ST && (BS == 2048 || BS == 4096) && (k >= 2 || std::is_same<IN, float>::value) && (ulcx_pattern(wc) >> 4) == 0
                         && ovFirst == BS && nextOv >= BS;
#endif
    if (fastBlk) nnz = (BS == 2048) ? xf_fast<IN, 2048, AN>(c, lds, s, k, blk, tid) : xf_fast<IN, 4096, AN>(c, lds, s, k, blk, tid);
    else
    for (int ch0 = 0; ch0 < C; ch0 += 2) {
        const int nch = ST ? 2 : ((ch0 + 1 < C) ? 2 : 1);
        unsigned pat = ulcx_pattern(wc);
        int off = 0, ovL = ovFirst;
        do {
            int S = BS >> (pat & 7);
            int d = pat & 7;
            pat >>= 4;
            int ov;
            if (pat) { ov = BS >> (pat & 7); if (pat & 8) ov >>= (wc & 7); }
            else ov = nextOv;
            if (ov > S) ov = S;
            const int M = S >> 1;
            int t0 = (k - 1) * BS - BS / 2 + off - S / 2;
            int aL = (S - ovL) >> 1, aR = (S - ov) >> 1;
            const float *rise = c.T.winRise + ovL, *fall = c.T.winFall + ov;
            const float2 *pre = c.T.pre[d];
            const int Mp = FFT_PADDEDS(M, ps);
            float2 *zc0 = z, *zs0 = z + Mp, *zc1 = z + (AN ? 1 : 2) * Mp, *zs1 = z + 3 * Mp;

            if (twInLds) for (int i = tid; i < M / 2; i += WG) twl[i] = c.T.tw[d][i];
            auto fold = [&](auto inpcmT, auto fullovT) {
                constexpr bool INPCM = decltype(inpcmT)::value, FULLOV = decltype(fullovT)::value;
                const IN *frame = pcm_base<IN>(c) + ((size_t)s * c.K * BS + (INPCM ? t0 : 0)) * C;
                auto ldE = [&](int pos, int e) -> float { return INPCM ? ld1(frame + (size_t)pos * C + e) : smp_ld1<IN>(c, s, t0 + pos, e); };
                auto ldQ = [&](int pos) -> float4 { return INPCM ? ld4(frame + (size_t)pos * C) : smp_ld4<IN>(c, s, t0 + pos); };
                for (int jj = tid; jj < M / 2; jj += WG) {
                    const int iA = 2 * jj, iB = S - 2 - 2 * jj, iC = S + 2 * jj, iD = 2 * S - 2 - 2 * jj;
                    float2 xs[8];
                    {
                        const int ip[4] = { iA, iB, iC, iD };
#pragma unroll
                        for (int r = 0; r < 4; r++) {
                            float2 e0, e1;
                            if (nch == 2) {
                                if (C == 2) { float4 v = ldQ(ip[r]); e0 = make_float2(v.x, v.y); e1 = make_float2(v.z, v.w); }
                                else { e0 = make_float2(ldE(ip[r], ch0), ldE(ip[r], ch0 + 1)); e1 = make_float2(ldE(ip[r] + 1, ch0), ldE(ip[r] + 1, ch0 + 1)); }
                                xs[2 * r]     = make_float2((e0.x + e0.y) * 0.5f, (e0.x - e0.y) * 0.5f);
                                xs[2 * r + 1] = make_float2((e1.x + e1.y) * 0.5f, (e1.x - e1.y) * 0.5f);
                            } else {
                                xs[2 * r] = make_float2(ldE(ip[r], ch0), 0.0f); xs[2 * r + 1] = make_float2(ldE(ip[r] + 1, ch0), 0.0f);
                            }
                        }
                    }
                    const int ipos[8] = { iA, iA + 1, iB, iB + 1, iC, iC + 1, iD, iD + 1 };
#pragma unroll
                    for (int r = 0; r < 8; r++) {
                        if (FULLOV) {
                            float f = (r < 4) ? rise[ipos[r]] : fall[ipos[r] - S];
                            xs[r].x *= f; xs[r].y *= f;
                            continue;
                        }
                        float f; bool zero;
                        if (r < 4) {
                            int idx = ipos[r] - aL;
                            int ci = idx < 0 ? 0 : (idx < ovL ? idx : 0);
                            float tv = rise[ci];
                            f = (idx < ovL) ? tv : 1.0f; zero = idx < 0;
                        } else {
                            int idx = ipos[r] - S - aR;
                            int ci = idx < 0 ? 0 : (idx < ov ? idx : 0);
                            float tv = fall[ci];
                            f = (idx < 0) ? 1.0f : tv; zero = idx >= ov;
                        }
                        float wx = xs[r].x * f, wy = xs[r].y * f;
                        xs[r].x = zero ? 0.0f : wx;
                        xs[r].y = zero ? 0.0f : wy;
                    }
#pragma unroll
                    for (int hsel = 0; hsel < 2; hsel++) {
                        const int n = hsel ? M / 2 + jj : M / 2 - 1 - jj;
                        const float2 lbv = hsel ? xs[0] : xs[1], lav = hsel ? xs[3] : xs[2];
                        const float2 rav = hsel ? xs[4] : xs[5], rbv = hsel ? xs[7] : xs[6];
                        float2 P = pre[n];
#pragma unroll
                        for (int q = 0; q < 2; q++) {
                            if (q >= nch) break;
                            float ra = q ? rav.y : rav.x, rb = q ? rbv.y : rbv.x, la = q ? lav.y : lav.x, lb = q ? lbv.y : lbv.x;
                            float vr = ra + rb, wr = ra - rb;
                            float vl = la - lb, wl = lb + la;
                            float v1 = hsel ? vl : vr, v2 = hsel ? vr : vl;
                            float w1 = hsel ? wl : wr, w2 = hsel ? wr : wl;
                            float2 *zc = q ? zc1 : zc0, *zs = q ? zs1 : zs0;
                            zc[FFT_PADS(n, ps)] = cmulc(make_float2(v1, v2), P);
                            if constexpr (!AN) zs[FFT_PADS(n, ps)] = cmulc(make_float2(w2, w1), P);
                        }
                    }
                }
            };
            if (!(ULCX_DBG(c) & 2)) {
                const bool inPcm = (t0 >= 0), fullOv = (ovL == S) && (ov == S);
                if (inPcm && fullOv) fold(std::true_type{}, std::true_type{});
                else if (inPcm) fold(std::true_type{}, std::false_type{});
                else fold(std::false_type{}, std::false_type{});
            }
            __syncthreads();

            if (!(ULCX_DBG(c) & 1)) for (int a = __builtin_amdgcn_readfirstlane(tid >> 6); a < (AN ? 1 : 2) * nch; a += WG / 64) {
                if (twInLds) fft_wave_dif(z + a * Mp, M, twl, tid & 63, ps);
                else fft_wave_dif(z + a * Mp, M, c.T.tw[d], tid & 63, ps);
            }
            __syncthreads();

            int bits = 31 - __clz(M);
            float norm = 2.0f / S;
            if (!(ULCX_DBG(c) & 4)) for (int kk = tid; kk < M / 2; kk += WG) {
                int k1 = kk, k2 = M - 1 - kk;
                int r1 = (int)(__brev((unsigned)k1) >> (32 - bits));
                int r2 = (int)(__brev((unsigned)k2) >> (32 - bits));
                float2 P1 = pre[k1], P2 = pre[k2];
                float am1 = 0.0f, am2 = 0.0f;
                if (ampLds) { am1 = amp2[off / 2 + k1]; am2 = amp2[off / 2 + k2]; }
#pragma unroll
                for (int q = 0; q < 2; q++) {
                    if (q >= nch) break;
                    int ch = ch0 + q;
                    float2 *zc = q ? zc1 : zc0, *zs = q ? zs1 : zs0;
                    const fft_v2f Pv1 = { P1.x, P1.y }, Pv2 = { P2.x, P2.y };
                    auto cm = [](float2 d, fft_v2f w) { const fft_v2f dv = { d.x, d.y }; const fft_v2f r = fft_cmulc_post_pk(dv, w); return make_float2(r.x, r.y); };
                    float2 yc1 = cm(zc[FFT_PADS(r1, ps)], Pv1), yc2 = cm(zc[FFT_PADS(r2, ps)], Pv2);
                    if constexpr (AN) {
                        const float mdctA[4] = { yc1.x, yc2.y, yc2.x, yc1.y };
#pragma unroll
                        for (int p = 0; p < 2; p++) {
                            const int j = p ? k2 : k1;
                            stnt((float2 *)(coefO + (size_t)ch * BS + off + 2 * j), make_float2(mdctA[2*p] * norm, mdctA[2*p+1] * norm));
                        }
                        continue;
                    }
                    float2 ys1 = cm(zs[FFT_PADS(r1, ps)], Pv1), ys2 = cm(zs[FFT_PADS(r2, ps)], Pv2);
                    float mdct[4] = { yc1.x, yc2.y, yc2.x, yc1.y };
                    float mdst[4] = { ys1.x, ys2.y, ys2.x, ys1.y };
#pragma unroll
                    for (int p = 0; p < 2; p++) {
                        float re0 = mdct[2*p] * norm,   im0 = mdst[2*p] * norm;
                        float re1 = mdct[2*p+1] * norm, im1 = mdst[2*p+1] * norm;
                        float re0s = re0 * re0, im0s = im0 * im0, re1s = re1 * re1, im1s = im1 * im1;
                        float a0 = re0s + im0s, a1 = re1s + im1s;
                        nnz += (fabsf(re0) < 0.5f * ULCX_COEF_EPS) ? 0 : 1;
                        nnz += (fabsf(re1) < 0.5f * ULCX_COEF_EPS) ? 0 : 1;
                        int j = p ? k2 : k1;
                        size_t gi = (size_t)ch * BS + off + 2 * j;
                        stnt((float2 *)(coefO + gi), make_float2(re0, re1));
                        stnt(c.nsum + tile_idx(BS / 2, blk * C + ch, off / 2 + j), a0 + a1);
                        if (p) { am2 += a0; am2 += a1; } else { am1 += a0; am1 += a1; }
                    }
                }
                if (AN) continue;
                if (ampLds) { amp2[off / 2 + k1] = am1; amp2[off / 2 + k2] = am2; }
                else { c.amp2[tile_idx(BS / 2, blk, off / 2 + k1)] = am1; c.amp2[tile_idx(BS / 2, blk, off / 2 + k2)] = am2; }
            }
            __syncthreads();
            off += S; ovL = ov;
        } while (pat);
    }
    if (AN) return;
    for (int o = 32; o > 0; o >>= 1) nnz += __shfl_down(nnz, o);
    if ((tid & 63) == 0) atomicAdd(&s_nnz, nnz);
    if (ampLds) for (int i = tid; i < BS / 2; i += WG) c.amp2[tile_idx(BS / 2, blk, i)] = amp2[i];
    __syncthreads();
    if (tid == 0) c.nnz[blk] = s_nnz;
}

#ifndef ULCX_XF_ANALYSIS_UNIT
template <bool ST, typename IN>
__global__ __launch_bounds__(WG, 4) void k_xf(UlcxEncCtx c, int k0, int k1) {
    extern __shared__ float lds[];
    const int kc = k1 - k0;
    const int NBk = c.B * kc;
    const int per = (NBk + 7) / 8;
    const int vb = (int)(blockIdx.x % 8) * per + (int)(blockIdx.x / 8);
    if (vb >= NBk) return;
    xf_block<ST, IN>(c, lds, vb / kc, k0 + vb % kc, threadIdx.x);
}
#else
template <bool ST, typename IN>
__global__ __launch_bounds__(WG, XFA_LB) void k_xfa(UlcxEncCtx c, int k0, int k1) {
    extern __shared__ float lds[];
    const int kc = k1 - k0;
    const int NBk = c.B * kc;
    const int per = (NBk + 7) / 8;
    const int vb = (int)(blockIdx.x % 8) * per + (int)(blockIdx.x / 8);
    if (vb >= NBk) return;
    xf_block<ST, IN, true>(c, lds, vb / kc, k0 + vb % kc, threadIdx.x);
}
#endif

template <typename IN, bool AN>
__device__ __forceinline__ void xf_big_block(const UlcxEncCtx &c, int k0, int k1) {
    extern __shared__ float lds[];
    const int BS = c.BS, C = c.C;
    const int kc = k1 - k0;
    const int NBk = c.B * kc;
    const int vb = blockIdx.x;
    if (vb >= NBk) return;
    const int s = vb / kc, k = k0 + vb % kc;
    const int blk = s * c.K + k;
    const int tid = threadIdx.x;
    float2 *z = (float2 *)lds;
    __shared__ int s_nnz;
    if (tid == 0) s_nnz = 0;
    const int *wrow = c.wcArr + (size_t)s * (c.maxK + 2) + k;
    const int wcPrev = wrow[0], wc = wrow[1], wcNext = wrow[2];
    if (!AN && c.barkRing && threadIdx.x == 0 && (ulcx_pattern(wc) & ~8u) != 0) c.decList[atomicAdd(c.decCount, 1)] = blk;
    const int nextOv = first_overlap(wcNext, BS);
    int ovFirst;
    {
        unsigned pp = ulcx_pattern(wcPrev);
        int lastS = BS;
        do { lastS = BS >> (pp & 7); } while (pp >>= 4);
        ovFirst = first_overlap(wc, BS);
        if (ovFirst > lastS) ovFirst = lastS;
    }
    const size_t cb = (size_t)C * BS;
    float *coefO = c.coef + (size_t)blk * cb;
    int nnz = 0;
    __syncthreads();
    for (int ch = 0; ch < C; ch++) {
        unsigned pat = ulcx_pattern(wc);
        int off = 0, ovL = ovFirst;
        do {
            const int S = BS >> (pat & 7);
            const int d = pat & 7;
            pat >>= 4;
            int ov;
            if (pat) { ov = BS >> (pat & 7); if (pat & 8) ov >>= (wc & 7); }
            else ov = nextOv;
            if (ov > S) ov = S;
            const int M = S >> 1;
            const int t0 = (k - 1) * BS - BS / 2 + off - S / 2;
            const int aL = (S - ovL) >> 1, aR = (S - ov) >> 1;
            const float *rise = c.T.winRise + ovL, *fall = c.T.winFall + ov;
            const float2 *pre = c.T.pre[d];
            const int bits = 31 - __clz(M);
            const float norm = 2.0f / S;
            for (int kind = 0; kind < (AN ? 1 : 2); kind++) {
                for (int jj = tid; jj < M / 2; jj += WG) {
                    const int iA = 2 * jj, iB = S - 2 - 2 * jj, iC = S + 2 * jj, iD = 2 * S - 2 - 2 * jj;
                    const int ipos[8] = { iA, iA + 1, iB, iB + 1, iC, iC + 1, iD, iD + 1 };
                    float xs[8];
#pragma unroll
                    for (int r = 0; r < 8; r++) xs[r] = win_apply(ms_sample<IN>(c, s, t0 + ipos[r], ch), ipos[r], S, aL, ovL, aR, ov, rise, fall);
#pragma unroll
                    for (int hsel = 0; hsel < 2; hsel++) {
                        const int n = hsel ? M / 2 + jj : M / 2 - 1 - jj;
                        const float lb = hsel ? xs[0] : xs[1], la = hsel ? xs[3] : xs[2];
                        const float ra = hsel ? xs[4] : xs[5], rb = hsel ? xs[7] : xs[6];
                        const float vr = ra + rb, wr = ra - rb;
                        const float vl = la - lb, wl = lb + la;
                        const float v1 = hsel ? vl : vr, v2 = hsel ? vr : vl;
                        const float w1 = hsel ? wl : wr, w2 = hsel ? wr : wl;
                        z[n] = kind ? cmulc(make_float2(w2, w1), pre[n]) : cmulc(make_float2(v1, v2), pre[n]);
                    }
                }
                __syncthreads();
                fftn_dif(z, 1, M, c.T.tw[d], tid);
                for (int kk = tid; kk < M / 2; kk += WG) {
                    const int kA = kk, kB = M - 1 - kk;
                    const int r1 = (int)(__brev((unsigned)kA) >> (32 - bits));
                    const int r2 = (int)(__brev((unsigned)kB) >> (32 - bits));
                    const float2 y1 = cmulc_post(z[r1], pre[kA]), y2 = cmulc_post(z[r2], pre[kB]);
#pragma unroll
                    for (int p = 0; p < 2; p++) {
                        const int j = p ? kB : kA;
                        const size_t gi = (size_t)ch * BS + off + 2 * j;
                        if (kind == 0) {
                            const float m0 = p ? y2.x : y1.x, m1 = p ? y1.y : y2.y;
                            const float re0 = m0 * norm, re1 = m1 * norm;
                            nnz += (fabsf(re0) < 0.5f * ULCX_COEF_EPS) ? 0 : 1;
                            nnz += (fabsf(re1) < 0.5f * ULCX_COEF_EPS) ? 0 : 1;
                            *(float2 *)(coefO + gi) = make_float2(re0, re1);
                        } else {
                            const float m0 = p ? y2.x : y1.x, m1 = p ? y1.y : y2.y;
                            const float im0 = m0 * norm, im1 = m1 * norm;
                            const float2 re = *(const float2 *)(coefO + gi);
                            const float re0s = re.x * re.x, im0s = im0 * im0, re1s = re.y * re.y, im1s = im1 * im1;
                            const float a0 = re0s + im0s, a1 = re1s + im1s;
                            c.nsum[tile_idx(BS / 2, blk * C + ch, off / 2 + j)] = a0 + a1;
                            float *ap = c.amp2 + tile_idx(BS / 2, blk, off / 2 + j);
                            float am = (ch == 0) ? 0.0f : *ap;
                            am += a0; am += a1;
                            *ap = am;
                        }
                    }
                }
                __syncthreads();
            }
            off += S; ovL = ov;
        } while (pat);
    }
    if (AN) return;
    for (int o = 32; o > 0; o >>= 1) nnz += __shfl_down(nnz, o);
    if ((tid & 63) == 0) atomicAdd(&s_nnz, nnz);
    __syncthreads();
    if (tid == 0) c.nnz[blk] = s_nnz;
}

#ifndef ULCX_XF_ANALYSIS_UNIT
template <typename IN>
__global__ __launch_bounds__(WG) void k_xf_big(UlcxEncCtx c, int k0, int k1) {
    xf_big_block<IN, false>(c, k0, k1);
}
#else
template <typename IN>
__global__ __launch_bounds__(WG) void k_xfa_big(UlcxEncCtx c, int k0, int k1) {
    xf_big_block<IN, true>(c, k0, k1);
}
#endif

#ifndef ULCX_XF_ANALYSIS_UNIT
__global__ __launch_bounds__(64) void k_cplx(UlcxEncCtx c, int k0, int k1) {
    const int gidc = blockIdx.x * 64 + threadIdx.x, kcc = k1 - k0;
    if (gidc >= c.B * kcc) return;
    const int blk = (gidc / kcc) * c.K + k0 + gidc % kcc;
    int n = c.C * c.BS;
    const float4 *p = (const float4 *)(c.coef + (size_t)blk * n);
    float cx = 0.0f, cw = 0.0f;
    int tiny = 0;
    auto sums = [&](auto tinyT) {
        constexpr bool TINY = decltype(tinyT)::value;
        for (int i = 0; i < n / 4; i += 4) {
            float4 q[4];
#pragma unroll
            for (int u = 0; u < 4; u++) q[u] = p[i + u];
#pragma unroll
            for (int u = 0; u < 4; u++) {
                float4 v = q[u];
                cx += v.x * v.x; cw += fabsf(v.x);
                cx += v.y * v.y; cw += fabsf(v.y);
                cx += v.z * v.z; cw += fabsf(v.z);
                cx += v.w * v.w; cw += fabsf(v.w);
                if (TINY) {
                    tiny += (fabsf(v.x) >= 0.5f * ULCX_COEF_EPS && fabsf(v.x) < 0x1.0p-29f) ? 1 : 0;
                    tiny += (fabsf(v.y) >= 0.5f * ULCX_COEF_EPS && fabsf(v.y) < 0x1.0p-29f) ? 1 : 0;
                    tiny += (fabsf(v.z) >= 0.5f * ULCX_COEF_EPS && fabsf(v.z) < 0x1.0p-29f) ? 1 : 0;
                    tiny += (fabsf(v.w) >= 0.5f * ULCX_COEF_EPS && fabsf(v.w) < 0x1.0p-29f) ? 1 : 0;
                }
            }
        }
    };
    int mode = c.mode;
    float p0 = c.p0, p1 = c.p1, vbrTarget = c.vbrTarget;
    if (c.rates) {
        const float2 r = c.rates[blk / c.K];
        if (r.x < 0.0f) {
            mode = ULCX_MODE_VBR; p0 = -r.x;
            vbrTarget = 0x1.E4EFB7p3f * ulcx_logf(100.0f / p0);
        } else { mode = (r.y > 0.0f) ? ULCX_MODE_ABR : ULCX_MODE_CBR; p0 = r.x; p1 = r.y; }
        if (__ballot(mode != ULCX_MODE_VBR)) sums(std::true_type{}); else sums(std::false_type{});
    } else if (c.mode == ULCX_MODE_VBR) sums(std::false_type{}); else sums(std::true_type{});
    if (cx != 0.0f) {
        cx = ulcx_logf((cw * cw) / cx) / c.cplxScale;
        if (cx < 0.0f) cx = 0.0f;
        if (cx > 1.0f) cx = 1.0f;
    }
    c.cplx[blk] = cx;
    int maxCoef = c.nnz[blk];
    if (mode == ULCX_MODE_VBR) {
        int nT = maxCoef;
        if (vbrTarget > 0.0f) {
            float ft = (c.C * c.BS) * cx / vbrTarget;
            if (ft < maxCoef) nT = (int)ft;
        }
        c.nout[blk] = nT;
        if (c.rates) {
            c.cbrLo[blk] = 0; c.cbrHi[blk] = maxCoef;
            c.cbrDone[blk] = ULCX_DONE_VBR;
            c.cbrBudget[blk] = 0;
            c.selWin[blk] = make_uint4(0u, 0u, (uint32_t)(c.C * c.BS), 0u);
            for (int u = 0; u < c.C * 4; u++) c.tailSum[((size_t)blk * c.C * 4 + u) * 8 + 6] = 0.0f;
        }
    } else {
        float kbps = p0;
        if (mode == ULCX_MODE_ABR) kbps = p0 * cx / p1;
        int budget = (int)((c.BS * kbps) * 1000.0f / c.rateHz);
        int lo = 0, hi = maxCoef;
        int done = (0 < maxCoef) ? 0 : 1;
        int nOut = (0 < maxCoef) ? (int)((unsigned)(0 + maxCoef) / 2u) : 0;
        while (!done && 4 * (nOut - tiny + 1) > budget) {
            hi = nOut - 1;
            if (!(lo < hi - 1)) { done = 1; nOut = lo; }
            else nOut = (int)((unsigned)(lo + hi) / 2u);
        }
        c.cbrLo[blk] = lo; c.cbrHi[blk] = hi;
        c.cbrDone[blk] = done;
        c.selWin[blk] = make_uint4(0u, 0u, (uint32_t)(c.C * c.BS), 0u);
        for (int u = 0; u < c.C * 4; u++) c.tailSum[((size_t)blk * c.C * 4 + u) * 8 + 6] = 0.0f;
        {
            const unsigned long long open = __ballot(!done);
            if (open && (int)__builtin_amdgcn_mbcnt_hi((uint32_t)(open >> 32), __builtin_amdgcn_mbcnt_lo((uint32_t)open, 0u)) == 0 && !done)
                atomicAdd(c.cbrLive, (int)__popcll(open));
        }
        c.nout[blk] = nOut;
        c.cbrBudget[blk] = budget;
    }
    c.isFb[blk] = 0;
    if (c.useWave) c.slow[blk] = 0;
    if (blk == 0) { *c.fbCount = 0; if (c.useWave) { c.slow[c.B * c.K] = 0; c.slow[c.B * c.K + 1] = 0; } }
    int s = blk / c.K, k = blk % c.K;
    if (c.wcOut)   c.wcOut[blk]   = c.wcArr[(size_t)s * (c.maxK + 2) + k + 1];
    if (c.cplxOut) c.cplxOut[blk] = cx;
}

#else
__global__ __launch_bounds__(64) void k_cplxa(UlcxEncCtx c, int k0, int k1) {
    const int gidc = blockIdx.x * 64 + threadIdx.x, kcc = k1 - k0;
    if (gidc >= c.B * kcc) return;
    const int s = gidc / kcc, k = k0 + gidc % kcc;
    const int blk = s * c.K + k;
    if (c.wcOut) c.wcOut[blk] = c.wcArr[(size_t)s * (c.maxK + 2) + k + 1];
    if (!c.cplxOut) return;
    const int n = c.C * c.BS;
    const float4 *p = (const float4 *)(c.coef + (size_t)blk * n);
    float cx = 0.0f, cw = 0.0f;
    for (int i = 0; i < n / 4; i += 4) {
        float4 q[4];
#pragma unroll
        for (int u = 0; u < 4; u++) q[u] = p[i + u];
#pragma unroll
        for (int u = 0; u < 4; u++) {
            float4 v = q[u];
            cx += v.x * v.x; cw += fabsf(v.x);
            cx += v.y * v.y; cw += fabsf(v.y);
            cx += v.z * v.z; cw += fabsf(v.z);
            cx += v.w * v.w; cw += fabsf(v.w);
        }
    }
    if (cx != 0.0f) {
        cx = ulcx_logf((cw * cw) / cx) / c.cplxScale;
        if (cx < 0.0f) cx = 0.0f;
        if (cx > 1.0f) cx = 1.0f;
    }
    c.cplxOut[blk] = cx;
}
#endif

#ifndef ULCX_XF_ANALYSIS_UNIT
template <typename IN>
__global__ __launch_bounds__(WG) void k_state_update(UlcxEncCtx c) {
    int s = blockIdx.x, tid = threadIdx.x;
    int n = 2 * c.BS * c.C;
    float *h = c.hist + (size_t)s * n;
    int newF = c.K * c.BS * c.C;
    const IN *p = pcm_base<IN>(c) + (size_t)s * newF;
    if (c.K >= 2) {
        for (int i = tid; i < n; i += WG) h[i] = ld1(p + newF - n + i);
    } else {
        int half = n / 2;
        for (int i = tid; i < half; i += WG) { h[i] = h[half + i]; h[half + i] = ld1(p + i); }
    }
    if (tid == 0) {
        UlcxWcState &w = c.wcs[s];
        const int *row = c.wcArr + (size_t)s * (c.maxK + 2);
        w.wcPrev = row[c.K];
        w.wcCur = row[c.K + 1];
        const float *bins = c.bins + ((size_t)s * (c.maxK + 1) + c.K) * 16;
        for (int i = 0; i < 8; i++) { w.binSum[i] = bins[i]; w.binW[i] = bins[8 + i]; }
    }
}

template __global__ void k_xf<false, float>(UlcxEncCtx, int, int);
template __global__ void k_xf<false, int16_t>(UlcxEncCtx, int, int);
template __global__ void k_xf<true, float>(UlcxEncCtx, int, int);
template __global__ void k_xf<true, int16_t>(UlcxEncCtx, int, int);
template __global__ void k_xf_big<float>(UlcxEncCtx, int, int);
template __global__ void k_xf_big<int16_t>(UlcxEncCtx, int, int);
template __global__ void k_state_update<float>(UlcxEncCtx);
template __global__ void k_state_update<int16_t>(UlcxEncCtx);
#else
template __global__ void k_xfa<false, float>(UlcxEncCtx, int, int);
template __global__ void k_xfa<false, int16_t>(UlcxEncCtx, int, int);
template __global__ void k_xfa<true, float>(UlcxEncCtx, int, int);
template __global__ void k_xfa<true, int16_t>(UlcxEncCtx, int, int);
template __global__ void k_xfa_big<float>(UlcxEncCtx, int, int);
template __global__ void k_xfa_big<int16_t>(UlcxEncCtx, int, int);
#endif
```

### ulc-codec_amd/csrc/ulcx_internal.h

```cpp
#pragma once
#include <hip/hip_runtime.h>
#include <stdint.h>
#include "../../include/ulc_amd.h"

#ifndef ULCX_DSYN_TWL
#define ULCX_DSYN_TWL 1
#endif
#define ULCX_NBARK 25
#define ULCX_MAX_SUB 4
#define ULCX_BARK_EVENTS 52
#define ULCX_MAX_BS_DEVICE 32768
#define ULCX_COEF_EPS (0x1.0p-31f)
#define ULCX_HEAP_LDS_BYTES (128 * 1024)
#define ULCX_HEAP_GRID 256
#define ULCX_DONE_VBR 2
#ifdef ULCX_ABLATE
#define ULCX_DBG(c) ((c).dbgSkip)
#else
#define ULCX_DBG(c) 0
#endif

struct UlcxTables {
    const float2 *pre[ULCX_MAX_SUB];
    const float2 *tw[ULCX_MAX_SUB];
    const float  *winFall;
    const float  *winRise;
    const int    *bandIdx[ULCX_MAX_SUB];
    const float  *bandFrac[ULCX_MAX_SUB];
    const float4 *bandW[ULCX_MAX_SUB];
    const uint32_t *barkSched;
    short nBeg[ULCX_MAX_SUB][ULCX_NBARK], nEnd[ULCX_MAX_SUB][ULCX_NBARK];
    short pBeg[ULCX_MAX_SUB][ULCX_NBARK], pEnd[ULCX_MAX_SUB][ULCX_NBARK];
};

struct UlcxWcState {
    float tf[3];
    int   wcPrev, wcCur;
    float binSum[8], binW[8];
    int   pad;
};

struct UlcxEncCtx {
    int B, K, C, BS, lgBS;
    int barkRing;
    int *decList, *decCount;
    int maxK;
    int slot;
    int unitCap;
    int mode; float p0, p1;
    float vbrTarget;
    const float2 *rates;
    float cHP, cBP, qHP, qBP, cBlk;
    float cplxScale;
    int   rateHz;
    UlcxTables T;
    int keyFinal;
    const float *pcm; const int16_t *pcm16;
    uint8_t *out; int32_t *bits; int32_t *wcOut; float *cplxOut;
    float *hist;
    UlcxWcState *wcs;
    float2 *env;
    float  *bins;
    int    *wcArr;
    float  *coef;
    float  *key;
    float  *nsum;
    float  *npair;
    float  *amp2;
    float  *barkN;
    float  *barkP;
    double *barkRawN, *barkRawP;
    int    *nnz;
    float  *cplx;
    int    *nout;
    int    *cbrLo, *cbrHi, *cbrDone;
    uint32_t *keep;
    int    *fbList; int *fbCount;
    uint8_t *unitBuf;
    int    *unitNyb;
    int    *cbrBudget;
    uint4  *selWin;
    uint32_t *selT;
    int     selPair;
    int     selPass;
    int    *cbrLive;
    int    *slow;
    float2 *gapSum;
    float  *tailSum;
    int     useGapSums;
    int    *isFb;
    int    *ownSlot;
    int    *rankBuf;
    int     dbgSkip;
    int     forceFb;
    int     rankSlots, fbLo, fbHi;
    int     fbMode;
    int     useWave;
    int     directPack;
    void   *heapScratch;
};

struct UlcxDecCtx {
    int B, K, C, BS, lgBS, maxK;
    int s0, s1;
    int slot;
    int dbgSkip;
    UlcxTables T;
    const uint8_t *in; float *pcm; int16_t *pcm16;
    long long inBytes;
    int32_t *bits;
    float *lap;
    int   *lastSub;
    uint32_t *seed;
    int   *dead;
    float *lapO; int *lastSubO; uint32_t *seedO; int *deadO;
    float *lapScratch;
    int    synFull;
    int    k0, k1;
    int   *wcScan;
    int   *draws;
    int   *unitDraws;
    float4 *unitTail;
    int4  *unitRec;
    uint2 *prec; int precStride;
    uint2 *nrec; int nrecStride;
    float *tailMag;
    int    tailStride;
    float *scratch;
    const uint32_t *jumpT;
    const uint32_t *parT;
    int    fastOK, twInLds;
    int   packed;
    long long payStride;
    const int32_t *payBytes;
    int  *packOff;
    int  *blkOff;
    int   range;
    const ulcx_index_entry *rIndex;
    int   rIndexStride;
    const int32_t *rIndexBlocks, *rFirst;
    int2 *rInfo;
    int32_t *bitsOut;
};

__host__ __device__ static inline unsigned ulcx_pattern(int wc) {
    const unsigned i = ((unsigned)wc >> 4) & 15u;
    const unsigned long long t0 = 0x0091001900080000ull, t1 = 0x0A2102A101A2012Aull, t2 = 0x1B3213B212B3123Bull, t3 = 0xB3213B212B3123B1ull;
    const unsigned long long t = (i & 8u) ? ((i & 4u) ? t3 : t2) : ((i & 4u) ? t1 : t0);
    return (unsigned)(t >> (16u * (i & 3u))) & 0xFFFFu;
}

int  ulcx_tables_build(UlcxTables *devT, void **devBlob, int BS, int rateHz, bool forEncoder);
void ulcx_set_error(const char *fmt, ...);

#define ULCX_ENC_STAGES 20
#define ULCX_ENC_STAGES_REPORTED (ULCX_ENC_STAGES + 1)
extern const char *const ulcx_enc_stage_names[ULCX_ENC_STAGES_REPORTED];
#define ULCX_DEC_STAGES 2
#define ULCX_WC_MAXCH 32
#define ULCX_XF_MAXCH 8
#define ULCX_LDS_LIMIT (160 * 1024)
struct UlcxEncSync {
    hipEvent_t wcStart, wcForward[ULCX_WC_MAXCH], wcBackward[ULCX_WC_MAXCH], wcDecided[ULCX_WC_MAXCH];
    hipEvent_t xfChunkDone[ULCX_XF_MAXCH], cplxChunksDone;
    hipEvent_t noiseFork, noiseDone, tailFork, tailDone;
    hipEvent_t cplxDone, stateDone;
    hipEvent_t exactFork, exactFork2, exactJoin;
    hipEvent_t xfTiming[2 * ULCX_XF_MAXCH];
    hipStream_t side, side2, side3;
};
struct UlcxEncAux {
    UlcxEncSync &sync;
    int wcPipe;
    int wcSteps, wcFuse, nsSlots;
    int &nXf;
};
int ulcx_enc_launch(const UlcxEncCtx &c, hipStream_t st, hipEvent_t *ev , const UlcxEncAux &aux);
int ulcx_enc_launch_ladder(const UlcxEncCtx *rungs, int nRungs, hipStream_t st, hipEvent_t *ev, const UlcxEncAux &aux);
void ulcx_enc_rung_arm(const UlcxEncCtx &c, hipStream_t st);
struct UlcxDecAux {
    int synGrid;
    int synFull;
};
int ulcx_dec_launch(const UlcxDecCtx &c, hipStream_t st, hipEvent_t *ev, const UlcxDecAux &aux);
int ulcx_index_launch(const UlcxDecCtx &c, int maxBlocks, ulcx_index_entry *d_index, int32_t *d_nBlocks, hipStream_t st);
size_t ulcx_dec_lds_bytes(int BS, int fast, int twInLds);
int ulcx_dec_syn_slots(const UlcxDecCtx &c);
int ulcx_pack_launch(int nStreams, int nBlocks, int slotBytes, const uint8_t *d_slots, const int32_t *d_bits, uint8_t *d_payload,
                     long long stride, int32_t *d_payloadBytes, int32_t *d_maxBlock, hipStream_t st);
int ulcx_analyse_launch(const UlcxEncCtx &c, hipStream_t st, hipEvent_t *ev, const UlcxEncAux &aux, int useKxf);
int ulcx_enc_nsums_slots(int BS, int C);
__host__ __device__ static inline int ulcx_xf_pad_shift(int BS, int C) { (void)BS; (void)C; return 4; }
#define ULCX_SEL_CAP 8
#ifndef ULCX_SEL_CAND
#define ULCX_SEL_CAND 128
#endif
__host__ __device__ static inline int ulcx_sel_lds_words(int BS) { int a = BS / 2 + 4 * ULCX_NBARK, b = ULCX_SEL_CAP * 64; return a > b ? a : b; }
struct UlcxSlotRows {
    uint8_t *hdr; size_t hdrStride;
    uint8_t *big; size_t bigStride;
    uint8_t *small[4]; size_t smallStride;
};
struct UlcxSlotGeom {
    int B;
    int rowVec;
    int isEnc, nSmall, smallWords;
    int padWords;
    uint4 header;
};
int ulcx_slots_gather(const UlcxSlotRows &obj, const UlcxSlotRows &rows, const int32_t *d_slots, int n, const UlcxSlotGeom &g, hipStream_t st);
int ulcx_slots_scatter(const UlcxSlotRows &obj, const UlcxSlotRows &rows, const int32_t *d_slots, int n, const UlcxSlotGeom &g, hipStream_t st);
int ulcx_slots_reset(const UlcxSlotRows &obj, const int32_t *d_slots, int n, const UlcxSlotGeom &g, hipStream_t st);
void ulcx_enc_finalize_keys(const UlcxEncCtx &c, hipStream_t st);
void ulcx_enc_materialise_noise(const UlcxEncCtx &c, hipStream_t st);
```

### ulc-codec_amd/ulc_amd.py

```python
import ctypes as C
import os
import numpy as np

_HERE = os.path.dirname(os.path.abspath(__file__))
LIB_PATH = os.environ.get("ULC_AMD_LIB") or os.path.join(_HERE, "libulc_amd.so")

MODE_VBR, MODE_CBR, MODE_ABR = 0, 1, 2
_f32p = C.POINTER(C.c_float)
_i32p = C.POINTER(C.c_int32)
_u8p = C.POINTER(C.c_uint8)

EXPORTS = [
    "ULC_EncoderState_Init", "ULC_EncoderState_Destroy", "ULC_EncodeBlock_CBR", "ULC_EncodeBlock_ABR",
    "ULC_EncodeBlock_VBR", "ULC_DecoderState_Init", "ULC_DecoderState_Destroy", "ULC_DecodeBlock",
    "ulcx_last_error", "ulcx_device_count", "ulcx_encoder_create", "ulcx_encoder_destroy", "ulcx_encoder_reset",
    "ulcx_encoder_slot_bytes", "ulcx_encode_dev", "ulcx_encode_dev_pcm16", "ulcx_encode_host", "ulcx_encoder_debug_fetch",
    "ulcx_decoder_create", "ulcx_decoder_destroy", "ulcx_decoder_reset", "ulcx_decode_dev", "ulcx_decode_dev_pcm16", "ulcx_decode_host",
    "ulcx_encoder_last_fallbacks", "ulcx_encoder_debug_force_exact", "ulcx_ulc_header_pack", "ulcx_ulc_header_parse", "ulcx_ulc_rate_kbps",
    "ulcx_pack_streams_dev", "ulcx_decode_packed_dev", "ulcx_decode_packed_host", "ulcx_decoder_upload_payload", "ulcx_decode_resident_host", "ulcx_encoder_stage_ms", "ulcx_encoder_stage_name", "ulcx_encoder_last_xf_launches", "ulcx_decoder_stage_ms", "ulcx_decoder_stage_name", "ulcx_block_extent_bytes", "ulcx_encoder_set_timing", "ulcx_decoder_set_timing", "ulcx_encode_block1", "ulcx_decode_block1", "ulcx_decode_block1_rng", "ulcx_build_rev", "ulcx_dec_split_plan", "ulcx_dec_tail_plan", "ulcx_decoder_last_cut",
    "ulcx_encode_dev_rates", "ulcx_encode_dev_pcm16_rates", "ulcx_encode_host_rates",
    "ulcx_analyse_dev", "ulcx_analyse_dev_pcm16", "ulcx_analyse_host",
    "ulcx_index_packed_dev", "ulcx_index_packed_host", "ulcx_decode_range_dev", "ulcx_decode_range_dev_pcm16", "ulcx_decode_range_host",
    "ulcx_decoder_index_resident", "ulcx_decode_resident_range_host", "ulcx_dec_range_tail_plan",
    "ulcx_encode_dev_ladder", "ulcx_encode_dev_pcm16_ladder", "ulcx_encode_host_ladder", "ulcx_encoder_last_rungs",
    "ulcx_encoder_stream_state_bytes", "ulcx_decoder_stream_state_bytes",
    "ulcx_encoder_reset_streams_dev", "ulcx_encoder_save_streams_dev", "ulcx_encoder_load_streams_dev",
    "ulcx_decoder_reset_streams_dev", "ulcx_decoder_save_streams_dev", "ulcx_decoder_load_streams_dev",
    "ulcx_encoder_reset_streams_host", "ulcx_encoder_save_streams_host", "ulcx_encoder_load_streams_host",
    "ulcx_decoder_reset_streams_host", "ulcx_decoder_save_streams_host", "ulcx_decoder_load_streams_host",
    "ulcx_encode_dev_subset", "ulcx_encode_dev_pcm16_subset", "ulcx_analyse_dev_subset", "ulcx_encode_host_subset",
    "ulcx_decode_dev_subset", "ulcx_decode_dev_pcm16_subset", "ulcx_decode_host_subset",
]

MAX_RUNGS = 8

INDEX_DTYPE = np.dtype([("ByteOffs", np.int32), ("RngState", np.uint32)])



class FileHeader(C.Structure):
    _fields_ = [("Magic", C.c_uint32), ("BlockSize", C.c_uint16), ("MaxBlockSize", C.c_uint16), ("nBlocks", C.c_uint32),
                ("RateHz", C.c_uint32), ("nChan", C.c_uint16), ("RateKbps", C.c_uint16), ("StreamOffs", C.c_uint32)]


class Rung(C.Structure):
    _fields_ = [("mode", C.c_int32), ("param0", C.c_float), ("param1", C.c_float), ("reserved", C.c_int32), ("rate", C.c_void_p)]


_lib = None


def lib():
    global _lib
    if _lib is None:
        if not os.path.exists(LIB_PATH):
            raise RuntimeError(f"{LIB_PATH} not built: run `make -C ulc-codec_amd` (or __graft_entry__.build())")
        l = C.CDLL(LIB_PATH)
        l.ulcx_last_error.restype = C.c_char_p
        l.ulcx_build_rev.restype = C.c_char_p
        l.ulcx_encoder_create.argtypes = [C.POINTER(C.c_void_p), C.c_int, C.c_int, C.c_int, C.c_int, C.c_int, C.c_int]
        l.ulcx_encoder_destroy.argtypes = [C.c_void_p]
        l.ulcx_encoder_reset.argtypes = [C.c_void_p]
        l.ulcx_encoder_slot_bytes.argtypes = [C.c_void_p]
        l.ulcx_encode_dev.argtypes = [C.c_void_p, C.c_int, C.c_float, C.c_float, C.c_void_p, C.c_int,
                                      C.c_void_p, C.c_void_p, C.c_void_p, C.c_void_p, C.c_void_p]
        l.ulcx_encode_dev_pcm16.argtypes = l.ulcx_encode_dev.argtypes
        l.ulcx_encode_host.argtypes = [C.c_void_p, C.c_int, C.c_float, C.c_float, _f32p, C.c_int, _u8p, _i32p, _i32p, _f32p]
        if hasattr(l, "ulcx_encode_dev_rates"):
            l.ulcx_encode_dev_rates.argtypes = [C.c_void_p, C.c_void_p, C.c_void_p, C.c_int, C.c_void_p, C.c_void_p, C.c_void_p, C.c_void_p, C.c_void_p]
            l.ulcx_encode_dev_pcm16_rates.argtypes = l.ulcx_encode_dev_rates.argtypes
            l.ulcx_encode_host_rates.argtypes = [C.c_void_p, _f32p, _f32p, C.c_int, _u8p, _i32p, _i32p, _f32p]
        if hasattr(l, "ulcx_analyse_dev"):
            l.ulcx_analyse_dev.argtypes = [C.c_void_p, C.c_void_p, C.c_int, C.c_void_p, C.c_void_p, C.c_void_p]
            l.ulcx_analyse_dev_pcm16.argtypes = l.ulcx_analyse_dev.argtypes
            l.ulcx_analyse_host.argtypes = [C.c_void_p, _f32p, C.c_int, _i32p, _f32p]
        if hasattr(l, "ulcx_index_packed_dev"):
            l.ulcx_index_packed_dev.argtypes = [C.c_void_p, C.c_void_p, C.c_longlong, C.c_void_p, C.c_int, C.c_void_p, C.c_void_p, C.c_void_p]
            l.ulcx_index_packed_host.argtypes = [C.c_void_p, _u8p, C.c_longlong, _i32p, C.c_int, C.c_void_p, _i32p]
            l.ulcx_decode_range_dev.argtypes = [C.c_void_p, C.c_void_p, C.c_longlong, C.c_void_p, C.c_void_p, C.c_int, C.c_void_p, C.c_void_p, C.c_int,
                                                C.c_void_p, C.c_void_p, C.c_void_p]
            l.ulcx_decode_range_dev_pcm16.argtypes = l.ulcx_decode_range_dev.argtypes
            l.ulcx_decode_range_host.argtypes = [C.c_void_p, _u8p, C.c_longlong, _i32p, C.c_void_p, C.c_int, _i32p, _i32p, C.c_int, _f32p, _i32p]
            l.ulcx_decoder_index_resident.argtypes = [C.c_void_p, C.c_int, _i32p]
            l.ulcx_dec_range_tail_plan.argtypes = [C.c_int, C.c_int, C.c_int, _i32p]
            l.ulcx_decode_resident_range_host.argtypes = [C.c_void_p, _i32p, C.c_int, _f32p, _i32p]
        if hasattr(l, "ulcx_encode_dev_ladder"):
            l.ulcx_encode_dev_ladder.argtypes = [C.c_void_p, C.POINTER(Rung), C.c_int, C.c_void_p, C.c_int, C.c_void_p, C.c_void_p, C.c_void_p, C.c_void_p, C.c_void_p]
            l.ulcx_encode_dev_pcm16_ladder.argtypes = l.ulcx_encode_dev_ladder.argtypes
            l.ulcx_encode_host_ladder.argtypes = [C.c_void_p, C.POINTER(Rung), C.c_int, _f32p, C.c_int, _u8p, _i32p, _i32p, _f32p]
            l.ulcx_encoder_last_rungs.argtypes = [C.c_void_p]
        if hasattr(l, "ulcx_encode_dev_subset"):
            for kind in ("encoder", "decoder"):
                getattr(l, f"ulcx_{kind}_stream_state_bytes").restype = C.c_size_t
                getattr(l, f"ulcx_{kind}_stream_state_bytes").argtypes = [C.c_void_p]
                getattr(l, f"ulcx_{kind}_reset_streams_dev").argtypes = [C.c_void_p, C.c_void_p, C.c_int, C.c_void_p]
                getattr(l, f"ulcx_{kind}_save_streams_dev").argtypes = [C.c_void_p, C.c_void_p, C.c_int, C.c_void_p, C.c_void_p]
                getattr(l, f"ulcx_{kind}_load_streams_dev").argtypes = [C.c_void_p, C.c_void_p, C.c_int, C.c_void_p, C.c_void_p]
                getattr(l, f"ulcx_{kind}_reset_streams_host").argtypes = [C.c_void_p, _i32p, C.c_int]
                getattr(l, f"ulcx_{kind}_save_streams_host").argtypes = [C.c_void_p, _i32p, C.c_int, _u8p]
                getattr(l, f"ulcx_{kind}_load_streams_host").argtypes = [C.c_void_p, _i32p, C.c_int, _u8p]
            l.ulcx_encode_dev_subset.argtypes = [C.c_void_p, C.c_void_p, C.c_int, C.c_int, C.c_float, C.c_float, C.c_void_p, C.c_void_p, C.c_int,
                                                 C.c_void_p, C.c_void_p, C.c_void_p, C.c_void_p, C.c_void_p]
            l.ulcx_encode_dev_pcm16_subset.argtypes = l.ulcx_encode_dev_subset.argtypes
            l.ulcx_analyse_dev_subset.argtypes = [C.c_void_p, C.c_void_p, C.c_int, C.c_void_p, C.c_int, C.c_void_p, C.c_void_p, C.c_void_p]
            l.ulcx_encode_host_subset.argtypes = [C.c_void_p, _i32p, C.c_int, C.c_int, C.c_float, C.c_float, _f32p, _f32p, C.c_int,
                                                  _u8p, _i32p, _i32p, _f32p]
            l.ulcx_decode_dev_subset.argtypes = [C.c_void_p, C.c_void_p, C.c_int, C.c_void_p, C.c_int, C.c_int, C.c_void_p, C.c_void_p, C.c_void_p]
            l.ulcx_decode_dev_pcm16_subset.argtypes = l.ulcx_decode_dev_subset.argtypes
            l.ulcx_decode_host_subset.argtypes = [C.c_void_p, _i32p, C.c_int, _u8p, C.c_int, C.c_int, _f32p, _i32p]
        l.ulcx_encoder_debug_fetch.argtypes = [C.c_void_p, C.c_int, _f32p, _f32p, _f32p, _u8p, _i32p]
        l.ulcx_decoder_create.argtypes = [C.POINTER(C.c_void_p), C.c_int, C.c_int, C.c_int, C.c_int, C.c_int]
        l.ulcx_decoder_destroy.argtypes = [C.c_void_p]
        l.ulcx_decoder_reset.argtypes = [C.c_void_p]
        l.ulcx_decode_dev.argtypes = [C.c_void_p, C.c_void_p, C.c_int, C.c_int, C.c_void_p, C.c_void_p, C.c_void_p]
        l.ulcx_decode_dev_pcm16.argtypes = l.ulcx_decode_dev.argtypes
        l.ulcx_decode_host.argtypes = [C.c_void_p, _u8p, C.c_int, C.c_int, _f32p, _i32p]
        l.ulcx_encoder_last_fallbacks.argtypes = [C.c_void_p]
        l.ulcx_decoder_last_cut.argtypes = [C.c_void_p, _i32p, _i32p, _i32p]
        l.ulcx_dec_tail_plan.argtypes = [C.c_int, C.c_int, C.c_int, _i32p]
        l.ulcx_encoder_debug_force_exact.argtypes = [C.c_void_p, C.c_int]
        l.ulcx_decode_packed_dev.argtypes = [C.c_void_p, C.c_void_p, C.c_longlong, C.c_void_p, C.c_int, C.c_void_p, C.c_void_p, C.c_void_p]
        l.ulcx_decode_packed_host.argtypes = [C.c_void_p, _u8p, C.c_longlong, _i32p, C.c_int, _f32p, _i32p]
        l.ulcx_encoder_set_timing.argtypes = [C.c_void_p, C.c_int]
        l.ulcx_decoder_set_timing.argtypes = [C.c_void_p, C.c_int]
        l.ulcx_decoder_upload_payload.argtypes = [C.c_void_p, _u8p, C.c_longlong, _i32p]
        l.ulcx_decode_resident_host.argtypes = [C.c_void_p, C.c_int, _f32p, _i32p]
        l.ulcx_pack_streams_dev.argtypes = [C.c_int, C.c_int, C.c_int, C.c_int, C.c_void_p, C.c_void_p, C.c_void_p, C.c_longlong,
                                            C.c_void_p, C.c_void_p, C.c_void_p]
        l.ulcx_ulc_header_pack.argtypes = [_u8p, C.POINTER(FileHeader)]
        l.ulcx_ulc_header_parse.argtypes = [C.POINTER(FileHeader), _u8p, C.c_size_t]
        l.ulcx_ulc_rate_kbps.argtypes = [C.c_uint64, C.c_uint32, C.c_uint32, C.c_uint32]
        l.ulcx_encoder_stage_ms.argtypes = [C.c_void_p, _f32p, C.c_int]
        l.ulcx_encoder_last_xf_launches.argtypes = [C.c_void_p]
        l.ulcx_decoder_stage_ms.argtypes = [C.c_void_p, _f32p, C.c_int]
        l.ulcx_block_extent_bytes.argtypes = [C.c_void_p, C.c_int, C.c_int, C.c_int]
        l.ulcx_encoder_stage_name.restype = C.c_char_p
        l.ulcx_decoder_stage_name.restype = C.c_char_p
        _lib = l
    return _lib


class UlcError(RuntimeError):
    pass


def build_rev():
    return lib().ulcx_build_rev().decode()


def _check(rc, what):
    if rc != 0:
        raise UlcError(f"{what} failed ({rc}): {lib().ulcx_last_error().decode()}")


def _p(a, t):
    return a.ctypes.data_as(t) if a is not None else None


class _StreamSlots:
    _kind = None

    def _fn(self, what):
        return getattr(lib(), f"ulcx_{self._kind}_{what}"), f"ulcx_{self._kind}_{what}"

    @staticmethod
    def _slots(slots):
        s = np.ascontiguousarray(slots, dtype=np.int32).reshape(-1)
        return s, _p(s, _i32p)

    @property
    def state_bytes(self):
        return int(self._fn("stream_state_bytes")[0](self.h))

    def reset_streams(self, slots):
        s, sp = self._slots(slots)
        fn, name = self._fn("reset_streams_host")
        _check(fn(self.h, sp, s.size), name)

    def save_streams(self, slots):
        s, sp = self._slots(slots)
        state = np.zeros((s.size, self.state_bytes), np.uint8)
        fn, name = self._fn("save_streams_host")
        _check(fn(self.h, sp, s.size, _p(state, _u8p)), name)
        return state

    def load_streams(self, slots, state):
        s, sp = self._slots(slots)
        state = np.ascontiguousarray(state, dtype=np.uint8)
        assert state.size == s.size * self.state_bytes
        fn, name = self._fn("load_streams_host")
        _check(fn(self.h, sp, s.size, _p(state, _u8p)), name)

    def reset_streams_dev(self, d_slots, n, stream=0):
        fn, name = self._fn("reset_streams_dev")
        _check(fn(self.h, d_slots, n, stream or None), name)

    def save_streams_dev(self, d_slots, n, d_state, stream=0):
        fn, name = self._fn("save_streams_dev")
        _check(fn(self.h, d_slots, n, d_state, stream or None), name)

    def load_streams_dev(self, d_slots, n, d_state, stream=0):
        fn, name = self._fn("load_streams_dev")
        _check(fn(self.h, d_slots, n, d_state, stream or None), name)


class BatchEncoder(_StreamSlots):
    _kind = "encoder"

    def __init__(self, n_streams, n_chan, block_size, rate_hz, max_blocks, device=0):
        self.B, self.C, self.BS, self.rate, self.maxK = n_streams, n_chan, block_size, rate_hz, max_blocks
        self.h = C.c_void_p()
        _check(lib().ulcx_encoder_create(C.byref(self.h), device, n_streams, n_chan, block_size, rate_hz, max_blocks),
               "ulcx_encoder_create")
        self.slot = lib().ulcx_encoder_slot_bytes(self.h)
        self.lastK = 0

# ... 89 lines not shown
    def last_rungs(self):
        return int(lib().ulcx_encoder_last_rungs(self.h))

    def encode_dev(self, d_pcm, n_blocks, d_out, d_bits, d_wc=0, d_cplx=0, mode=MODE_VBR, p0=50.0, p1=0.0, stream=0):
        _check(lib().ulcx_encode_dev(self.h, mode, p0, p1, d_pcm, n_blocks, d_out, d_bits, d_wc or None, d_cplx or None,
                                     stream or None), "ulcx_encode_dev")
        self.lastK = n_blocks

    def encode_dev_pcm16(self, d_pcm16, n_blocks, d_out, d_bits, d_wc=0, d_cplx=0, mode=MODE_VBR, p0=50.0, p1=0.0, stream=0):
        _check(lib().ulcx_encode_dev_pcm16(self.h, mode, p0, p1, d_pcm16, n_blocks, d_out, d_bits, d_wc or None, d_cplx or None,
                                           stream or None), "ulcx_encode_dev_pcm16")
        self.lastK = n_blocks

    def analyse(self, pcm):
        pcm = np.ascontiguousarray(pcm, dtype=np.float32)
        assert pcm.shape[0] == self.B and pcm.shape[-1] == self.C
        K = pcm.shape[1] // self.BS
        assert pcm.shape[1] == K * self.BS
        wc = np.zeros((self.B, K), np.int32)
        cplx = np.zeros((self.B, K), np.float32)
        _check(lib().ulcx_analyse_host(self.h, _p(pcm, _f32p), K, _p(wc, _i32p), _p(cplx, _f32p)), "ulcx_analyse_host")
        self.lastK = K
        return wc, cplx

    def analyse_dev(self, d_pcm, n_blocks, d_wc=0, d_cplx=0, stream=0, pcm16=False):
        fn = lib().ulcx_analyse_dev_pcm16 if pcm16 else lib().ulcx_analyse_dev
        _check(fn(self.h, d_pcm, n_blocks, d_wc or None, d_cplx or None, stream or None),
               "ulcx_analyse_dev_pcm16" if pcm16 else "ulcx_analyse_dev")
        self.lastK = n_blocks

    def encode_subset(self, slots, pcm, mode=MODE_VBR, p0=50.0, p1=0.0, rates=None):
        s, sp = self._slots(slots)
        pcm = np.ascontiguousarray(pcm, dtype=np.float32)
        n = s.size
        assert pcm.shape[0] == n and pcm.shape[-1] == self.C
        K = pcm.shape[1] // self.BS
        assert pcm.shape[1] == K * self.BS
        if rates is not None:
            rates = np.ascontiguousarray(rates, dtype=np.float32)
            assert rates.shape == (n, 2)
        out = np.zeros((n, K, self.slot), np.uint8)
        bits = np.zeros((n, K), np.int32)
        wc = np.zeros((n, K), np.int32)
        cplx = np.zeros((n, K), np.float32)
        _check(lib().ulcx_encode_host_subset(self.h, sp, n, mode, p0, p1, _p(rates, _f32p), _p(pcm, _f32p), K, _p(out, _u8p),
                                             _p(bits, _i32p), _p(wc, _i32p), _p(cplx, _f32p)), "ulcx_encode_host_subset")
        self.lastK = K
        return out, bits, wc, cplx

    def encode_subset_dev(self, d_slots, n, d_pcm, n_blocks, d_out, d_bits, d_wc=0, d_cplx=0, mode=MODE_VBR, p0=50.0, p1=0.0, d_rates=0,
                          stream=0, pcm16=False):
        fn = lib().ulcx_encode_dev_pcm16_subset if pcm16 else lib().ulcx_encode_dev_subset
        _check(fn(self.h, d_slots, n, mode, p0, p1, d_rates or None, d_pcm, n_blocks, d_out, d_bits, d_wc or None, d_cplx or None,
                  stream or None), "ulcx_encode_dev_pcm16_subset" if pcm16 else "ulcx_encode_dev_subset")
        self.lastK = n_blocks

    def analyse_subset_dev(self, d_slots, n, d_pcm, n_blocks, d_wc=0, d_cplx=0, stream=0):
        _check(lib().ulcx_analyse_dev_subset(self.h, d_slots, n, d_pcm, n_blocks, d_wc or None, d_cplx or None, stream or None),
               "ulcx_analyse_dev_subset")
        self.lastK = n_blocks

    def debug_fetch(self, K=None, parts=("coef", "noise", "keys", "keep", "nout")):
        K = K or self.lastK
        n = self.C * self.BS
        shapes = dict(coef=((self.B, K, n), np.float32), noise=((self.B, K, n), np.float32), keys=((self.B, K, n), np.float32),
                      keep=((self.B, K, n), np.uint8), nout=((self.B, K), np.int32))
        unknown = set(parts) - set(shapes)
        if unknown:
            raise ValueError(f"unknown taps: {sorted(unknown)}")
        r = {k: (np.zeros(*shapes[k]) if k in parts else None) for k in shapes}
        _check(lib().ulcx_encoder_debug_fetch(self.h, K, _p(r["coef"], _f32p), _p(r["noise"], _f32p), _p(r["keys"], _f32p),
                                              _p(r["keep"], _u8p), _p(r["nout"], _i32p)), "ulcx_encoder_debug_fetch")
        return r

    def last_fallbacks(self):
        return lib().ulcx_encoder_last_fallbacks(self.h)

    def force_exact(self, every):
        _check(lib().ulcx_encoder_debug_force_exact(self.h, int(every)), "ulcx_encoder_debug_force_exact")

    def xf_launches(self):
        return int(lib().ulcx_encoder_last_xf_launches(self.h))

    def set_timing(self, on):
        _check(lib().ulcx_encoder_set_timing(self.h, int(bool(on))), "ulcx_encoder_set_timing")

    def stage_ms(self):
        ms = np.zeros(32, np.float32)
        n = lib().ulcx_encoder_stage_ms(self.h, _p(ms, _f32p), 32)
        return {lib().ulcx_encoder_stage_name(i).decode(): float(ms[i]) for i in range(n)}


class BatchDecoder(_StreamSlots):
    _kind = "decoder"

    def __init__(self, n_streams, n_chan, block_size, max_blocks, device=0):
        self.B, self.C, self.BS, self.maxK = n_streams, n_chan, block_size, max_blocks
        self.h = C.c_void_p()
        _check(lib().ulcx_decoder_create(C.byref(self.h), device, n_streams, n_chan, block_size, max_blocks),
               "ulcx_decoder_create")

    def close(self):
        if self.h:
            lib().ulcx_decoder_destroy(self.h)
            self.h = C.c_void_p()

    def __del__(self):
        try:
            self.close()
        except Exception:
            pass

    def last_cut(self):
        g, f, r = C.c_int32(0), C.c_int32(0), C.c_int32(0)
        _check(lib().ulcx_decoder_last_cut(self.h, C.byref(g), C.byref(f), C.byref(r)), "ulcx_decoder_last_cut")
        return g.value, f.value, r.value

    def reset(self):
        _check(lib().ulcx_decoder_reset(self.h), "ulcx_decoder_reset")

    def decode(self, blocks):
        blocks = np.ascontiguousarray(blocks, dtype=np.uint8)
        B, K, slot = blocks.shape
        assert B == self.B
        pcm = np.zeros((B, K * self.BS, self.C), np.float32)
        bits = np.zeros((B, K), np.int32)
        _check(lib().ulcx_decode_host(self.h, _p(blocks, _u8p), slot, K, _p(pcm, _f32p), _p(bits, _i32p)), "ulcx_decode_host")
        return pcm, bits

    def decode_packed(self, payload, payload_bytes, n_blocks):
        payload = np.ascontiguousarray(payload, dtype=np.uint8)
        nbytes = np.ascontiguousarray(payload_bytes, dtype=np.int32)
        B, stride = payload.shape
        pcm = np.zeros((B, n_blocks * self.BS, self.C), np.float32)
        bits = np.zeros((B, n_blocks), np.int32)
        _check(lib().ulcx_decode_packed_host(self.h, _p(payload, _u8p), stride, _p(nbytes, _i32p), n_blocks, _p(pcm, _f32p), _p(bits, _i32p)),
               "ulcx_decode_packed_host")
        return pcm, bits

    def upload_payload(self, payload, payload_bytes):
        payload = np.ascontiguousarray(payload, dtype=np.uint8)
        nbytes = np.ascontiguousarray(payload_bytes, dtype=np.int32)
        _check(lib().ulcx_decoder_upload_payload(self.h, _p(payload, _u8p), payload.shape[1], _p(nbytes, _i32p)), "ulcx_decoder_upload_payload")

    def decode_resident(self, n_blocks):
        pcm = np.zeros((self.B, n_blocks * self.BS, self.C), np.float32)
        bits = np.zeros((self.B, n_blocks), np.int32)
        _check(lib().ulcx_decode_resident_host(self.h, n_blocks, _p(pcm, _f32p), _p(bits, _i32p)), "ulcx_decode_resident_host")
        return pcm, bits

    def index_packed(self, payload, payload_bytes, max_blocks):
        payload = np.ascontiguousarray(payload, dtype=np.uint8)
        nbytes = np.ascontiguousarray(payload_bytes, dtype=np.int32)
        B, stride = payload.shape
        assert B == self.B
        index = np.zeros((B, max_blocks + 1), INDEX_DTYPE)
        count = np.zeros(B, np.int32)
        _check(lib().ulcx_index_packed_host(self.h, _p(payload, _u8p), stride, _p(nbytes, _i32p), max_blocks, index.ctypes.data, _p(count, _i32p)),
               "ulcx_index_packed_host")
        return index, count

    def decode_range(self, payload, payload_bytes, index, index_blocks, first, n_blocks):
        payload = np.ascontiguousarray(payload, dtype=np.uint8)
        nbytes = np.ascontiguousarray(payload_bytes, dtype=np.int32)
        index = np.ascontiguousarray(index, dtype=INDEX_DTYPE)
        count = np.ascontiguousarray(index_blocks, dtype=np.int32)
# ... 67 lines not shown
```

Baseline: 55510 Msamples/s.

## Speculatively run fast-path MDCT for all blocks before window-control decisions

Adds a speculative transform kernel that computes the fast-path stereo MDCT for every block up front, before the window-control chunks resolve. A fix-up kernel then redoes only the blocks whose final window pattern is not fast-path. A device-side gate tracks how many blocks needed redoing and turns speculation off for later calls when that share exceeds a threshold. The goal is to take the transform off the critical path behind window control, at the cost of wasted work on mispredicted blocks, an extra launch and a device-side flag check.

```diff
diff --git a/include/ulc_amd.h b/include/ulc_amd.h
--- a/include/ulc_amd.h
+++ b/include/ulc_amd.h
@@ -224,6 +224,7 @@
 int  ulcx_decoder_set_timing(ulcx_decoder *dec, int on);
 const char *ulcx_encoder_stage_name(int stage);
 int  ulcx_encoder_last_xf_launches(ulcx_encoder *enc);
+int  ulcx_encoder_last_xf_spec(ulcx_encoder *enc, int *speculated, int *redone);
 int  ulcx_decoder_stage_ms(ulcx_decoder *dec, float *ms, int maxStages);
 const char *ulcx_decoder_stage_name(int stage);
 
diff --git a/ulc-codec_amd/csrc/ulcx_api.cpp b/ulc-codec_amd/csrc/ulcx_api.cpp
--- a/ulc-codec_amd/csrc/ulcx_api.cpp
+++ b/ulc-codec_amd/csrc/ulcx_api.cpp
@@ -53,9 +53,10 @@
     std::vector<void *> allocs;
     hipEvent_t ev[ULCX_ENC_STAGES + 1] = {};
     bool evOk = false, evRecorded = false, timing = true;
-    int lastK = 0;
+    int lastK = 0, lastB = 0;
     UlcxEncSync sync = {};
     int wcPipe = 1, nXf = 0;
+    int xfSpecLaunched = 0;
     bool keysFinal = false;
     int wcSteps = -1, wcFuse = 1;
     int nsSlots = 0;
@@ -153,14 +154,15 @@
 }
 
 static const size_t kEncSyncUntimed = offsetof(UlcxEncSync, xfTiming) / sizeof(hipEvent_t);
+static const size_t kEncSyncTimed = sizeof(UlcxEncSync::xfTiming) / sizeof(hipEvent_t);
 static void enc_sync_destroy(UlcxEncSync &s) {
     hipEvent_t *ev = &s.wcStart;
-    for (size_t i = 0; i < kEncSyncUntimed + 2 * ULCX_XF_MAXCH; i++) if (ev[i]) hipEventDestroy(ev[i]);
+    for (size_t i = 0; i < kEncSyncUntimed + kEncSyncTimed; i++) if (ev[i]) hipEventDestroy(ev[i]);
     for (hipStream_t st : { s.side, s.side2, s.side3 }) if (st) hipStreamDestroy(st);
     s = UlcxEncSync{};
 }
 static bool enc_sync_create(UlcxEncSync &s) {
-    static_assert(offsetof(UlcxEncSync, wcStart) == 0 && offsetof(UlcxEncSync, side) == (kEncSyncUntimed + 2 * ULCX_XF_MAXCH) * sizeof(hipEvent_t), "UlcxEncSync: events, then streams");
+    static_assert(offsetof(UlcxEncSync, wcStart) == 0 && offsetof(UlcxEncSync, side) == (kEncSyncUntimed + kEncSyncTimed) * sizeof(hipEvent_t), "UlcxEncSync: events, then streams");
     hipEvent_t *ev = &s.wcStart;
     bool ok = true;
     for (hipStream_t *st : { &s.side, &s.side2, &s.side3 }) ok = ok && hipStreamCreateWithFlags(st, hipStreamNonBlocking) == hipSuccess;
@@ -254,6 +256,13 @@
     DA(c.barkP, NB * 4 * ULCX_NBARK, true);
     if (c.barkRing) { DA(c.barkRawN, NB * nChan * ULCX_NBARK * 3, false); DA(c.barkRawP, NB * ULCX_NBARK * 3, false); DA(c.decList, NB, false); DA(c.decCount, 1, true); }
     DA(c.nnz, NB, true);
+    DA(c.xfSpec, 4, true);
+    {
+        const int open = 1;
+        CKR(hipMemcpy(c.xfSpec, &open, sizeof(int), hipMemcpyHostToDevice));
+        const char *ev = getenv("ULCX_XF_SPEC");
+        c.xfSpecMode = !ev ? -1 : (ev[0] != '0') ? 1 : 0;
+    }
     DA(c.cplx, NB, true);
     DA(c.nout, NB, true);
     DA(c.slow, 3 * NB + 2, true);
@@ -324,7 +333,7 @@
 
 static UlcxEncAux enc_aux(ulcx_encoder *e, int nBlocks) {
     const int wcPipe = (nBlocks >= 2 * e->wcPipe) ? e->wcPipe : (nBlocks >= 6 && e->wcPipe > 1 ? 3 : 1);
-    return UlcxEncAux{ e->sync, wcPipe, e->wcSteps, e->wcFuse, e->nsSlots, e->nXf };
+    return UlcxEncAux{ e->sync, wcPipe, e->wcSteps, e->wcFuse, e->nsSlots, e->nXf, e->xfSpecLaunched };
 }
 
 static int slots_list_bad(const char *who, const int32_t *d_slots, int n, int B) {
@@ -412,7 +421,7 @@
 }
 static int enc_call_done(ulcx_encoder *e, int rc, int nBlocks, bool analyse, int rungs) {
     e->evRecorded = (rc == ULCX_OK) && e->timing;
-    e->lastK = nBlocks;
+    e->lastK = nBlocks; e->lastB = e->B;
     e->keysFinal = false;
     e->lastAnalyse = analyse;
     e->lastRungs = rungs;
@@ -445,7 +454,9 @@
     const UlcxEncAux aux = enc_aux(e, nBlocks);
     const int rc = enc_launch_on(e, c, subset ? d_slots : nullptr, n, (hipStream_t)hipStream,
                                  [&](UlcxEncCtx &cc) { return ulcx_enc_launch(cc, (hipStream_t)hipStream, e->timing ? e->ev : nullptr, aux); });
-    return enc_call_done(e, rc, nBlocks, false, 1);
+    enc_call_done(e, rc, nBlocks, false, 1);
+    if (subset) e->lastB = n;
+    return rc;
 }
 extern "C" int ulcx_encode_dev(ulcx_encoder *e, int mode, float p0, float p1, const float *d_pcm, int nBlocks,
                                uint8_t *d_out, int32_t *d_bits, int32_t *d_wc, float *d_cplx, void *hipStream) {
@@ -755,6 +766,18 @@
 }
 
 extern "C" int ulcx_encoder_last_xf_launches(ulcx_encoder *e) { return (e && e->evRecorded) ? (e->nXf > 0 ? e->nXf : 1) : 0; }
+extern "C" int ulcx_encoder_last_xf_spec(ulcx_encoder *e, int *speculated, int *redone) {
+    if (!e) return refuse("ulcx_encoder_last_xf_spec", "no encoder");
+    int w[4] = { 0, 0, 0, e->lastAnalyse ? 0 : e->lastK * e->lastB };
+    if (e->xfSpecLaunched) {
+        CKR(hipSetDevice(e->device));
+        CKR(hipDeviceSynchronize());
+        CKR(hipMemcpy(w, e->ctx.xfSpec, sizeof(w), hipMemcpyDeviceToHost));
+    }
+    if (speculated) *speculated = w[2];
+    if (redone) *redone = w[3];
+    return ULCX_OK;
+}
 
 static void cleanup(ulcx_decoder *e) {
     if (!e) return;
diff --git a/ulc-codec_amd/csrc/ulcx_enc.hip b/ulc-codec_amd/csrc/ulcx_enc.hip
--- a/ulc-codec_amd/csrc/ulcx_enc.hip
+++ b/ulc-codec_amd/csrc/ulcx_enc.hip
@@ -31,6 +31,11 @@
     return mdctOnly ? k_xfa<false, IN> : k_xf<false, IN>;
 }
 static RangeKernel xf_fn(const UlcxEncCtx &c, bool mdctOnly) { return c.pcm16 ? xf_fn_in<int16_t>(c, mdctOnly) : xf_fn_in<float>(c, mdctOnly); }
+static CallKernel xf_spec_fn(const UlcxEncCtx &c) {
+    if (c.BS == 2048) return c.pcm16 ? k_xf_spec<int16_t, 2048> : k_xf_spec<float, 2048>;
+    return c.pcm16 ? k_xf_spec<int16_t, 4096> : k_xf_spec<float, 4096>;
+}
+static RangeKernel xf_fix_fn(const UlcxEncCtx &c) { return c.pcm16 ? k_xf_fix<int16_t> : k_xf_fix<float>; }
 
 template <int PASS> static PassKernel select_fn_pass(const UlcxEncCtx &c, bool pair, bool rates) {
 #define SEL(R, L) (rates ? (PassKernel)k_select_wave_rates<R, L, PASS> : (PassKernel)k_select_wave<R, L, PASS>)
@@ -85,14 +90,15 @@
     const int SG = (c.B + 63) / 64;
     const int nCh = aux.wcPipe;
     const bool mdctOnly = (what == ULCX_FRONT_ANALYSE);
-    const RangeKernel xf = (what == ULCX_FRONT_WC_ONLY) ? nullptr : xf_fn(c, mdctOnly);
+    const bool spec = what == ULCX_FRONT_ENCODE && nCh > 1 && c.C == 2 && (c.BS == 2048 || c.BS == 4096) && c.xfSpecMode != 0;
+    const RangeKernel xf = (what == ULCX_FRONT_WC_ONLY) ? nullptr : spec ? xf_fix_fn(c) : xf_fn(c, mdctOnly);
     const size_t lds = mdctOnly ? ulcx_enc_xfa_lds_bytes(c.BS, c.C) : ulcx_enc_xf_lds_bytes(c.BS, c.C);
     if (xf) TRY(allow_lds((const void *)xf, lds));
     auto transform = [&](int k0, int k1) {
         if (xf) hipLaunchKernelGGL(xf, dim3((unsigned)((c.B * (k1 - k0) + 7) / 8) * 8), dim3(WG), lds, st, c, k0, k1);
     };
     const bool wcFuse = c.C == 2 && aux.wcFuse;
-    aux.nXf = 0;
+    aux.nXf = 0; aux.xfSpecLaunched = 0;
     if (nCh <= 1) {
         if (wcFuse) { MARK(mk, st); launch_wc_ef(c, st, 0, c.K);                                                  MARK(mk, st); }
         else {
@@ -120,6 +126,13 @@
     for (int w = 0; w <= nW; w++) wcs[w] = sameCuts ? cut[w] : (int)((long long)c.K * w / nW);
     CK(hipEventRecord(sy.wcStart, st));
     CK(hipStreamWaitEvent(side, sy.wcStart, 0));
+    if (spec) {
+        const CallKernel xs = xf_spec_fn(c);
+        TRY(allow_lds((const void *)xs, lds));
+        if (mk.ev) CK(hipEventRecord(sy.xfTiming[2 * nCh], st));
+        hipLaunchKernelGGL(xs, dim3((unsigned)((c.B * c.K + 7) / 8) * 8), dim3(WG), lds, st, c);
+        if (mk.ev) CK(hipEventRecord(sy.xfTiming[2 * nCh + 1], st));
+    }
     int jx = 0;
     for (int w = 0; w < nW; w++) {
         const int k0 = wcs[w], k1 = wcs[w + 1], kc = k1 - k0;
@@ -146,7 +159,8 @@
             jx++;
         }
     }
-    aux.nXf = nCh;
+    aux.nXf = spec ? nCh + 1 : nCh;
+    aux.xfSpecLaunched = spec ? 1 : 0;
     MARK(mk, st);
     for (int j = 0; j < nCh; j++) {
         CK(hipStreamWaitEvent(side, sy.xfChunkDone[j], 0));
@@ -154,6 +168,7 @@
         if (what == ULCX_FRONT_ENCODE) hipLaunchKernelGGL(k_cplx, dim3((c.B * kc2 + 63) / 64), dim3(64), 0, side, c, cut[j], cut[j + 1]);
         else hipLaunchKernelGGL(k_cplxa, dim3((c.B * kc2 + 63) / 64), dim3(64), 0, side, c, cut[j], cut[j + 1]);
     }
+    if (spec) hipLaunchKernelGGL(k_xf_gate, dim3(1), dim3(1), 0, side, c);
     CK(hipEventRecord(sy.cplxChunksDone, side));
     return ULCX_OK;
 }
diff --git a/ulc-codec_amd/csrc/ulcx_enc_dev.h b/ulc-codec_amd/csrc/ulcx_enc_dev.h
--- a/ulc-codec_amd/csrc/ulcx_enc_dev.h
+++ b/ulc-codec_amd/csrc/ulcx_enc_dev.h
@@ -378,6 +378,17 @@
 extern template __global__ void k_xf_big<float>(UlcxEncCtx, int, int);
 extern template __global__ void k_xf_big<int16_t>(UlcxEncCtx, int, int);
 __global__ void k_cplx(UlcxEncCtx c, int k0, int k1);
+template <typename IN, int BSC>
+__global__ __launch_bounds__(WG, 4) void k_xf_spec(UlcxEncCtx c);
+extern template __global__ void k_xf_spec<float, 2048>(UlcxEncCtx);
+extern template __global__ void k_xf_spec<float, 4096>(UlcxEncCtx);
+extern template __global__ void k_xf_spec<int16_t, 2048>(UlcxEncCtx);
+extern template __global__ void k_xf_spec<int16_t, 4096>(UlcxEncCtx);
+template <typename IN>
+__global__ __launch_bounds__(WG, 4) void k_xf_fix(UlcxEncCtx c, int k0, int k1);
+extern template __global__ void k_xf_fix<float>(UlcxEncCtx, int, int);
+extern template __global__ void k_xf_fix<int16_t>(UlcxEncCtx, int, int);
+__global__ void k_xf_gate(UlcxEncCtx c);
 #ifndef XFA_LB
 #define XFA_LB 4
 #endif
diff --git a/ulc-codec_amd/csrc/ulcx_enc_xf.hip b/ulc-codec_amd/csrc/ulcx_enc_xf.hip
--- a/ulc-codec_amd/csrc/ulcx_enc_xf.hip
+++ b/ulc-codec_amd/csrc/ulcx_enc_xf.hip
@@ -1,4 +1,7 @@
 #include "ulcx_enc_dev.h"
+#if !defined(ULCX_XF_ANALYSIS_UNIT) && !defined(ULCX_XF_SPEC_UNIT)
+#define ULCX_XF_MAIN_UNIT
+#endif
 
 __device__ __forceinline__ int first_overlap(int wc, int BS) {
     unsigned p = ulcx_pattern(wc);
@@ -176,7 +179,7 @@
     return ovFirst == BS && first_overlap(wcNext, BS) >= BS;
 }
 
-template <bool ST, typename IN, bool AN = false>
+template <bool ST, typename IN, bool AN = false, bool FIX = false>
 __device__ __forceinline__ void xf_block(const UlcxEncCtx &c, float *lds, int s, int k, const int tid) {
     const int BS = c.BS, C = ST ? 2 : c.C;
     const int blk = s * c.K + k;
@@ -214,6 +217,10 @@
     const bool fastBlk = ST && (BS == 2048 || BS == 4096) && (k >= 2 || std::is_same<IN, float>::value) && (ulcx_pattern(wc) >> 4) == 0
                          && ovFirst == BS && nextOv >= BS;
 #endif
+    if constexpr (FIX) {
+        if (!fastBlk) { if (tid == 0) atomicAdd(c.xfSpec + 1, 1); }
+        else if (c.xfSpecMode > 0 || c.xfSpec[0] != 0) return;
+    }
     if (fastBlk) nnz = (BS == 2048) ? xf_fast<IN, 2048, AN>(c, lds, s, k, blk, tid) : xf_fast<IN, 4096, AN>(c, lds, s, k, blk, tid);
     else
     for (int ch0 = 0; ch0 < C; ch0 += 2) {
@@ -379,7 +386,7 @@
     if (tid == 0) c.nnz[blk] = s_nnz;
 }
 
-#ifndef ULCX_XF_ANALYSIS_UNIT
+#ifdef ULCX_XF_MAIN_UNIT
 template <bool ST, typename IN>
 __global__ __launch_bounds__(WG, 4) void k_xf(UlcxEncCtx c, int k0, int k1) {
     extern __shared__ float lds[];
@@ -390,7 +397,48 @@
     if (vb >= NBk) return;
     xf_block<ST, IN>(c, lds, vb / kc, k0 + vb % kc, threadIdx.x);
 }
-#else
+#elif defined(ULCX_XF_SPEC_UNIT)
+__device__ __forceinline__ bool xf_spec_on(const UlcxEncCtx &c) { return c.xfSpecMode > 0 || c.xfSpec[0] != 0; }
+
+template <typename IN, int BSC>
+__global__ __launch_bounds__(WG, 4) void k_xf_spec(UlcxEncCtx c) {
+    extern __shared__ float lds[];
+    if (!xf_spec_on(c)) return;
+    const int NBk = c.B * c.K;
+    const int per = (NBk + 7) / 8;
+    const int vb = (int)(blockIdx.x % 8) * per + (int)(blockIdx.x / 8);
+    if (vb >= NBk) return;
+    const int s = vb / c.K, k = vb % c.K, tid = threadIdx.x;
+    if (!std::is_same<IN, float>::value && k < 2) return;
+    int &s_nnz = *(int *)(lds + 4 * FFT_PADDEDS(BSC, 4) + BSC / 2);
+    if (tid == 0) s_nnz = 0;
+    int nnz = xf_fast<IN, BSC>(c, lds, s, k, vb, tid);
+    for (int o = 32; o > 0; o >>= 1) nnz += __shfl_down(nnz, o);
+    if ((tid & 63) == 0) atomicAdd(&s_nnz, nnz);
+    __syncthreads();
+    if (tid == 0) c.nnz[vb] = s_nnz;
+}
+
+template <typename IN>
+__global__ __launch_bounds__(WG, 4) void k_xf_fix(UlcxEncCtx c, int k0, int k1) {
+    extern __shared__ float lds[];
+    const int kc = k1 - k0;
+    const int NBk = c.B * kc;
+    const int per = (NBk + 7) / 8;
+    const int vb = (int)(blockIdx.x % 8) * per + (int)(blockIdx.x / 8);
+    if (vb >= NBk) return;
+    xf_block<true, IN, false, true>(c, lds, vb / kc, k0 + vb % kc, threadIdx.x);
+}
+
+__global__ void k_xf_gate(UlcxEncCtx c) {
+    const int total = c.B * c.K, nonFast = c.xfSpec[1];
+    const int on = xf_spec_on(c) ? 1 : 0;
+    c.xfSpec[2] = on;
+    c.xfSpec[3] = on ? nonFast : total;
+    c.xfSpec[0] = ((long long)nonFast * 1000 <= (long long)total * ULCX_XF_SPEC_GATE_PERMILLE) ? 1 : 0;
+    c.xfSpec[1] = 0;
+}
+#elif defined(ULCX_XF_ANALYSIS_UNIT)
 template <bool ST, typename IN>
 __global__ __launch_bounds__(WG, XFA_LB) void k_xfa(UlcxEncCtx c, int k0, int k1) {
     extern __shared__ float lds[];
@@ -513,19 +561,19 @@
     if (tid == 0) c.nnz[blk] = s_nnz;
 }
 
-#ifndef ULCX_XF_ANALYSIS_UNIT
+#ifdef ULCX_XF_MAIN_UNIT
 template <typename IN>
 __global__ __launch_bounds__(WG) void k_xf_big(UlcxEncCtx c, int k0, int k1) {
     xf_big_block<IN, false>(c, k0, k1);
 }
-#else
+#elif defined(ULCX_XF_ANALYSIS_UNIT)
 template <typename IN>
 __global__ __launch_bounds__(WG) void k_xfa_big(UlcxEncCtx c, int k0, int k1) {
     xf_big_block<IN, true>(c, k0, k1);
 }
 #endif
 
-#ifndef ULCX_XF_ANALYSIS_UNIT
+#ifdef ULCX_XF_MAIN_UNIT
 __global__ __launch_bounds__(64) void k_cplx(UlcxEncCtx c, int k0, int k1) {
     const int gidc = blockIdx.x * 64 + threadIdx.x, kcc = k1 - k0;
     if (gidc >= c.B * kcc) return;
@@ -619,7 +667,7 @@
     if (c.cplxOut) c.cplxOut[blk] = cx;
 }
 
-#else
+#elif defined(ULCX_XF_ANALYSIS_UNIT)
 __global__ __launch_bounds__(64) void k_cplxa(UlcxEncCtx c, int k0, int k1) {
     const int gidc = blockIdx.x * 64 + threadIdx.x, kcc = k1 - k0;
     if (gidc >= c.B * kcc) return;
@@ -652,7 +700,7 @@
 }
 #endif
 
-#ifndef ULCX_XF_ANALYSIS_UNIT
+#ifdef ULCX_XF_MAIN_UNIT
 template <typename IN>
 __global__ __launch_bounds__(WG) void k_state_update(UlcxEncCtx c) {
     int s = blockIdx.x, tid = threadIdx.x;
@@ -684,11 +732,18 @@
 template __global__ void k_xf_big<int16_t>(UlcxEncCtx, int, int);
 template __global__ void k_state_update<float>(UlcxEncCtx);
 template __global__ void k_state_update<int16_t>(UlcxEncCtx);
-#else
+#elif defined(ULCX_XF_ANALYSIS_UNIT)
 template __global__ void k_xfa<false, float>(UlcxEncCtx, int, int);
 template __global__ void k_xfa<false, int16_t>(UlcxEncCtx, int, int);
 template __global__ void k_xfa<true, float>(UlcxEncCtx, int, int);
 template __global__ void k_xfa<true, int16_t>(UlcxEncCtx, int, int);
 template __global__ void k_xfa_big<float>(UlcxEncCtx, int, int);
 template __global__ void k_xfa_big<int16_t>(UlcxEncCtx, int, int);
+#else
+template __global__ void k_xf_spec<float, 2048>(UlcxEncCtx);
+template __global__ void k_xf_spec<float, 4096>(UlcxEncCtx);
+template __global__ void k_xf_spec<int16_t, 2048>(UlcxEncCtx);
+template __global__ void k_xf_spec<int16_t, 4096>(UlcxEncCtx);
+template __global__ void k_xf_fix<float>(UlcxEncCtx, int, int);
+template __global__ void k_xf_fix<int16_t>(UlcxEncCtx, int, int);
 #endif
diff --git a/ulc-codec_amd/csrc/ulcx_enc_xfs.hip b/ulc-codec_amd/csrc/ulcx_enc_xfs.hip
--- /dev/null
+++ b/ulc-codec_amd/csrc/ulcx_enc_xfs.hip
@@ -0,0 +1,2 @@
+#define ULCX_XF_SPEC_UNIT
+#include "ulcx_enc_xf.hip"
diff --git a/ulc-codec_amd/csrc/ulcx_internal.h b/ulc-codec_amd/csrc/ulcx_internal.h
--- a/ulc-codec_amd/csrc/ulcx_internal.h
+++ b/ulc-codec_amd/csrc/ulcx_internal.h
@@ -45,6 +45,8 @@
     int barkRing;
     int *decList, *decCount;
     int maxK;
+    int *xfSpec;
+    int xfSpecMode;
     int slot;
     int unitCap;
     int mode; float p0, p1;
@@ -159,6 +161,7 @@
 #define ULCX_DEC_STAGES 2
 #define ULCX_WC_MAXCH 32
 #define ULCX_XF_MAXCH 8
+#define ULCX_XF_SPEC_GATE_PERMILLE 400
 #define ULCX_LDS_LIMIT (160 * 1024)
 struct UlcxEncSync {
     hipEvent_t wcStart, wcForward[ULCX_WC_MAXCH], wcBackward[ULCX_WC_MAXCH], wcDecided[ULCX_WC_MAXCH];
@@ -166,7 +169,7 @@
     hipEvent_t noiseFork, noiseDone, tailFork, tailDone;
     hipEvent_t cplxDone, stateDone;
     hipEvent_t exactFork, exactFork2, exactJoin;
-    hipEvent_t xfTiming[2 * ULCX_XF_MAXCH];
+    hipEvent_t xfTiming[2 * (ULCX_XF_MAXCH + 1)];
     hipStream_t side, side2, side3;
 };
 struct UlcxEncAux {
@@ -174,6 +177,7 @@
     int wcPipe;
     int wcSteps, wcFuse, nsSlots;
     int &nXf;
+    int &xfSpecLaunched;
 };
 int ulcx_enc_launch(const UlcxEncCtx &c, hipStream_t st, hipEvent_t *ev , const UlcxEncAux &aux);
 int ulcx_enc_launch_ladder(const UlcxEncCtx *rungs, int nRungs, hipStream_t st, hipEvent_t *ev, const UlcxEncAux &aux);
diff --git a/ulc-codec_amd/ulc_amd.py b/ulc-codec_amd/ulc_amd.py
--- a/ulc-codec_amd/ulc_amd.py
+++ b/ulc-codec_amd/ulc_amd.py
@@ -17,7 +17,7 @@
     "ulcx_encoder_slot_bytes", "ulcx_encode_dev", "ulcx_encode_dev_pcm16", "ulcx_encode_host", "ulcx_encoder_debug_fetch",
     "ulcx_decoder_create", "ulcx_decoder_destroy", "ulcx_decoder_reset", "ulcx_decode_dev", "ulcx_decode_dev_pcm16", "ulcx_decode_host",
     "ulcx_encoder_last_fallbacks", "ulcx_encoder_debug_force_exact", "ulcx_ulc_header_pack", "ulcx_ulc_header_parse", "ulcx_ulc_rate_kbps",
-    "ulcx_pack_streams_dev", "ulcx_decode_packed_dev", "ulcx_decode_packed_host", "ulcx_decoder_upload_payload", "ulcx_decode_resident_host", "ulcx_encoder_stage_ms", "ulcx_encoder_stage_name", "ulcx_encoder_last_xf_launches", "ulcx_decoder_stage_ms", "ulcx_decoder_stage_name", "ulcx_block_extent_bytes", "ulcx_encoder_set_timing", "ulcx_decoder_set_timing", "ulcx_encode_block1", "ulcx_decode_block1", "ulcx_decode_block1_rng", "ulcx_build_rev", "ulcx_dec_split_plan", "ulcx_dec_tail_plan", "ulcx_decoder_last_cut",
+    "ulcx_pack_streams_dev", "ulcx_decode_packed_dev", "ulcx_decode_packed_host", "ulcx_decoder_upload_payload", "ulcx_decode_resident_host", "ulcx_encoder_stage_ms", "ulcx_encoder_stage_name", "ulcx_encoder_last_xf_launches", "ulcx_encoder_last_xf_spec", "ulcx_decoder_stage_ms", "ulcx_decoder_stage_name", "ulcx_block_extent_bytes", "ulcx_encoder_set_timing", "ulcx_decoder_set_timing", "ulcx_encode_block1", "ulcx_decode_block1", "ulcx_decode_block1_rng", "ulcx_build_rev", "ulcx_dec_split_plan", "ulcx_dec_tail_plan", "ulcx_decoder_last_cut",
     "ulcx_encode_dev_rates", "ulcx_encode_dev_pcm16_rates", "ulcx_encode_host_rates",
     "ulcx_analyse_dev", "ulcx_analyse_dev_pcm16", "ulcx_analyse_host",
     "ulcx_index_packed_dev", "ulcx_index_packed_host", "ulcx_decode_range_dev", "ulcx_decode_range_dev_pcm16", "ulcx_decode_range_host",
@@ -132,6 +132,7 @@
         l.ulcx_ulc_rate_kbps.argtypes = [C.c_uint64, C.c_uint32, C.c_uint32, C.c_uint32]
         l.ulcx_encoder_stage_ms.argtypes = [C.c_void_p, _f32p, C.c_int]
         l.ulcx_encoder_last_xf_launches.argtypes = [C.c_void_p]
+        l.ulcx_encoder_last_xf_spec.argtypes = [C.c_void_p, C.POINTER(C.c_int), C.POINTER(C.c_int)]
         l.ulcx_decoder_stage_ms.argtypes = [C.c_void_p, _f32p, C.c_int]
         l.ulcx_block_extent_bytes.argtypes = [C.c_void_p, C.c_int, C.c_int, C.c_int]
         l.ulcx_encoder_stage_name.restype = C.c_char_p
@@ -387,6 +388,11 @@
     def xf_launches(self):
         return int(lib().ulcx_encoder_last_xf_launches(self.h))
 
+    def xf_spec(self):
+        spec, redone = C.c_int(0), C.c_int(0)
+        _check(lib().ulcx_encoder_last_xf_spec(self.h, C.byref(spec), C.byref(redone)), "ulcx_encoder_last_xf_spec")
+        return int(spec.value), int(redone.value)
+
     def set_timing(self, on):
         _check(lib().ulcx_encoder_set_timing(self.h, int(bool(on))), "ulcx_encoder_set_timing")
 
```

Result: slower. 47870 Msamples/s (-13.8%).
